# LPD-EPFL/ByzantineMomentum

Measured on AMD Instinct MI355X. Metric: aggregations/sec (Byzantine-robust GAR over n workers x d dims; achieved HBM GB/s per GAR in roofline/per_gar), higher is better.
Workload: dtype f32

## Files before the change

byzantinemomentum_amd/_lib.py:

```python

import ctypes
import pathlib

import torch

import os

_PKG_DIR = pathlib.Path(__file__).resolve().parent
LIB_PATH = pathlib.Path(os.environ["BM_GAR_LIB"]).resolve() if os.environ.get("BM_GAR_LIB") else _PKG_DIR / "libbm_gar.so"

ABI_VERSION = 23
MAX_ROWS = 64
EINVAL = -100000
ENOCOMM, ECOMM = -100001, -100002

OP_MEDIAN, OP_TRMEAN, OP_PHOCAS, OP_MEAMED = 0, 1, 2, 3
WS_PAIRWISE, WS_AKSEL, WS_STATS, WS_DOT, WS_STEP, WS_STUDY = 0, 1, 2, 3, 4, 5
STUDY_SLOTS = 32
STUDY_GRAM, STUDY_EX, STUDY_ATTACK = slice(0, 16), slice(16, 18), slice(18, 20)
STUDY_SUMS = slice(0, 20)
STUDY_MAXES = slice(20, 22)
STUDY_L2 = slice(22, 23)
OUT3_SUMS, OUT3_MAX = slice(0, 2), slice(2, 3)
STEP_S2, STEP_SD, STEP_H2, STEP_HD, STEP_D2, STEP_A2, STEP_AD, STEP_L2 = range(8)
STEP_GRAM, STEP_EX = slice(8, 24), slice(24, 26)
STEP_SMAX, STEP_HMAX, STEP_DMAX, STEP_AMAX = range(26, 30)
STEP_ACCEPT = 30
RANK_KRUM, RANK_BULYAN = 0, 1
ATTACK_EMPIRE, ATTACK_LITTLE, ATTACK_DIRECTION = 0, 1, 16

_c_float_pp = ctypes.POINTER(ctypes.c_void_p)

SIGNATURES = {
  "bm_abi_version": (ctypes.c_int, []),
  "bm_tuning_set": (ctypes.c_int, [ctypes.c_char_p, ctypes.c_int]),
  "bm_error_string": (ctypes.c_char_p, [ctypes.c_int]),
  "bm_colwise": (ctypes.c_int, [ctypes.c_int, _c_float_pp, ctypes.c_int, ctypes.c_int64, ctypes.c_int,
                                ctypes.c_void_p, ctypes.c_void_p]),
  "bm_workspace_bytes": (ctypes.c_int64, [ctypes.c_int, ctypes.c_int, ctypes.c_int64]),
  "bm_pairwise_sqdist": (ctypes.c_int, [_c_float_pp, ctypes.c_int, ctypes.c_int64, ctypes.c_void_p,
                                        ctypes.c_void_p, ctypes.c_void_p]),
  "bm_pairwise_sqdist_shard": (ctypes.c_int, [_c_float_pp, ctypes.c_int, ctypes.c_int64, ctypes.c_int64,
                                              ctypes.c_void_p, ctypes.c_void_p, ctypes.c_void_p]),
  "bm_krum_rank": (ctypes.c_int, [ctypes.c_void_p, ctypes.c_int, ctypes.c_int, ctypes.c_int, ctypes.c_int,
                                  ctypes.c_void_p, ctypes.c_void_p, ctypes.c_void_p]),
  "bm_selected_mean": (ctypes.c_int, [_c_float_pp, ctypes.c_int, ctypes.c_void_p, ctypes.c_int,
                                      ctypes.c_int64, ctypes.c_void_p, ctypes.c_void_p]),
  "bm_bulyan_pass2": (ctypes.c_int, [_c_float_pp, ctypes.c_int, ctypes.c_void_p, ctypes.c_int, ctypes.c_int,
                                     ctypes.c_int64, ctypes.c_void_p, ctypes.c_void_p]),
  "bm_aksel_pass1": (ctypes.c_int, [_c_float_pp, ctypes.c_int, ctypes.c_int64, ctypes.c_void_p,
                                    ctypes.c_void_p, ctypes.c_void_p, ctypes.c_void_p]),
  "bm_stack_stats": (ctypes.c_int, [_c_float_pp, ctypes.c_int, ctypes.c_int64, ctypes.c_void_p, ctypes.c_void_p,
                                    ctypes.c_float, ctypes.c_int, ctypes.c_void_p, ctypes.c_void_p,
                                    ctypes.c_void_p]),
  "bm_multi_dot": (ctypes.c_int, [_c_float_pp, ctypes.c_int, _c_float_pp, ctypes.c_int, ctypes.c_int64,
                                  ctypes.c_void_p, ctypes.c_void_p, ctypes.c_void_p]),
  "bm_momentum_stats_colwise": (ctypes.c_int, [_c_float_pp, ctypes.c_int, _c_float_pp, ctypes.c_int, ctypes.c_int64,
                                               ctypes.c_float, ctypes.c_float, ctypes.c_void_p, ctypes.c_void_p,
                                               ctypes.c_void_p, ctypes.c_void_p, ctypes.c_float, ctypes.c_int,
                                               ctypes.c_int, ctypes.c_int, ctypes.c_int, ctypes.c_void_p,
                                               ctypes.c_void_p, ctypes.c_void_p, ctypes.c_void_p]),
  "bm_momentum_stats_sqdist": (ctypes.c_int, [_c_float_pp, ctypes.c_int, _c_float_pp, ctypes.c_int, ctypes.c_int64,
                                              ctypes.c_int64, ctypes.c_float, ctypes.c_float, ctypes.c_void_p,
                                              ctypes.c_void_p, ctypes.c_void_p, ctypes.c_void_p, ctypes.c_float,
                                              ctypes.c_int, ctypes.c_int, ctypes.c_void_p, ctypes.c_void_p,
                                              ctypes.c_void_p, ctypes.c_void_p, ctypes.c_void_p]),
  "bm_sharded_sq_slot": (ctypes.c_void_p, [ctypes.c_void_p]),
  "bm_sharded_pair_workspace": (ctypes.c_void_p, [ctypes.c_void_p]),
  "bm_sharded_order_slot": (ctypes.c_void_p, [ctypes.c_void_p]),
  "bm_accept_count": (ctypes.c_int, [ctypes.c_void_p, ctypes.c_int, ctypes.c_int, ctypes.c_void_p, ctypes.c_void_p]),
  "bm_sharded_rule_from_sq": (ctypes.c_int, [ctypes.c_void_p, ctypes.c_int, _c_float_pp, ctypes.c_int, ctypes.c_int64,
                                             ctypes.c_int, ctypes.c_int, ctypes.c_void_p, ctypes.c_void_p,
                                             ctypes.c_void_p, ctypes.c_void_p]),
  "bm_stack_stats_colwise": (ctypes.c_int, [_c_float_pp, ctypes.c_int, ctypes.c_int64, ctypes.c_void_p, ctypes.c_void_p,
                                            ctypes.c_float, ctypes.c_int, ctypes.c_int, ctypes.c_int, ctypes.c_int,
                                            ctypes.c_void_p, ctypes.c_void_p, ctypes.c_void_p, ctypes.c_void_p]),
  "bm_stack_stats_sqdist": (ctypes.c_int, [_c_float_pp, ctypes.c_int, ctypes.c_int64, ctypes.c_int64, ctypes.c_void_p,
                                           ctypes.c_void_p, ctypes.c_float, ctypes.c_int, ctypes.c_int, ctypes.c_void_p,
                                           ctypes.c_void_p, ctypes.c_void_p, ctypes.c_void_p, ctypes.c_void_p]),
  "bm_study_stats": (ctypes.c_int, [ctypes.c_void_p, ctypes.c_void_p, ctypes.c_void_p, ctypes.c_void_p, ctypes.c_int,
                                    ctypes.c_void_p, ctypes.c_void_p, ctypes.c_void_p, ctypes.c_void_p, ctypes.c_int,
                                    ctypes.c_float, ctypes.c_float, ctypes.c_void_p, ctypes.c_void_p, ctypes.c_int64,
                                    ctypes.c_void_p, ctypes.c_void_p, ctypes.c_void_p]),
  "bm_study_stats_update": (ctypes.c_int, [ctypes.c_void_p, ctypes.c_void_p, ctypes.c_void_p, ctypes.c_void_p, ctypes.c_int,
                                           ctypes.c_void_p, ctypes.c_void_p, ctypes.c_void_p, ctypes.c_void_p, ctypes.c_int,
                                           ctypes.c_float, ctypes.c_float, ctypes.c_void_p, ctypes.c_void_p,
                                           ctypes.c_void_p, ctypes.c_float, ctypes.c_float, ctypes.c_int64,
                                           ctypes.c_void_p, ctypes.c_void_p, ctypes.c_void_p]),
  "bm_row_sqnorms": (ctypes.c_int, [_c_float_pp, ctypes.c_int, ctypes.c_int64, ctypes.c_void_p, ctypes.c_void_p,
                                    ctypes.c_void_p]),
  "bm_stable_argsort": (ctypes.c_int, [ctypes.c_void_p, ctypes.c_int, ctypes.c_void_p, ctypes.c_void_p]),
  "bm_anticge_workspace_bytes": (ctypes.c_int64, [ctypes.c_int64]),
  "bm_anticge_sum": (ctypes.c_int, [_c_float_pp, ctypes.c_int, ctypes.c_int64, ctypes.c_int, ctypes.c_void_p,
                                    ctypes.c_void_p, ctypes.c_void_p, ctypes.c_void_p, ctypes.c_void_p, ctypes.c_void_p]),
  "bm_anticge_scale": (ctypes.c_int, [ctypes.c_void_p, ctypes.c_int64, ctypes.c_void_p, ctypes.c_void_p]),
  "bm_attack_vector": (ctypes.c_int, [ctypes.c_int, ctypes.c_void_p, ctypes.c_int64, ctypes.c_int64, ctypes.c_float,
                                      ctypes.c_void_p, ctypes.c_void_p, ctypes.c_void_p, ctypes.c_void_p]),
  "bm_multi_axpby": (ctypes.c_int, [_c_float_pp, _c_float_pp, ctypes.c_int, ctypes.c_int64,
                                    ctypes.c_float, ctypes.c_float, ctypes.c_void_p]),
  "bm_brute_select": (ctypes.c_int, [ctypes.c_void_p, ctypes.c_int, ctypes.c_int, ctypes.c_void_p]),
  "bm_momentum_stats": (ctypes.c_int, [_c_float_pp, ctypes.c_int, _c_float_pp, ctypes.c_int, ctypes.c_int64,
                                       ctypes.c_float, ctypes.c_float, ctypes.c_void_p, ctypes.c_void_p,
                                       ctypes.c_void_p, ctypes.c_void_p, ctypes.c_float, ctypes.c_int,
                                       ctypes.c_void_p, ctypes.c_void_p, ctypes.c_void_p]),
  "bm_multi_fma3": (ctypes.c_int, [_c_float_pp, _c_float_pp, _c_float_pp, ctypes.c_int, ctypes.c_int64,
                                   ctypes.c_float, ctypes.c_float, ctypes.c_void_p, ctypes.c_void_p]),
  "bm_multi_fma3_bdev": (ctypes.c_int, [_c_float_pp, _c_float_pp, _c_float_pp, ctypes.c_int, ctypes.c_int64,
                                        ctypes.c_float, ctypes.c_void_p, ctypes.c_void_p, ctypes.c_void_p]),
  "bm_clip_factors": (ctypes.c_int, [ctypes.c_void_p, ctypes.c_int, ctypes.c_float, ctypes.c_void_p,
                                     ctypes.c_void_p]),
  "bm_multi_scale": (ctypes.c_int, [_c_float_pp, ctypes.c_int, ctypes.c_int64, ctypes.c_void_p, ctypes.c_void_p]),
  "bm_comm_available": (ctypes.c_int, []),
  "bm_comm_unique_id": (ctypes.c_int, [ctypes.c_void_p]),
  "bm_comm_init": (ctypes.c_int, [ctypes.POINTER(ctypes.c_void_p), ctypes.c_int, ctypes.c_int, ctypes.c_void_p]),
  "bm_comm_destroy": (ctypes.c_int, [ctypes.c_void_p]),
  "bm_comm_size": (ctypes.c_int, [ctypes.c_void_p]),
  "bm_allreduce_sum_f64": (ctypes.c_int, [ctypes.c_void_p, ctypes.c_void_p, ctypes.c_int64, ctypes.c_void_p]),
  "bm_allgather_f32": (ctypes.c_int, [ctypes.c_void_p, ctypes.c_void_p, ctypes.c_void_p, ctypes.c_int64,
                                      ctypes.c_void_p]),
  "bm_brute_select_device": (ctypes.c_int, [ctypes.c_void_p, ctypes.c_int, ctypes.c_int, ctypes.c_void_p, ctypes.c_void_p,
                                            ctypes.c_void_p]),
  "bm_colwise_eval_supported": (ctypes.c_int, [ctypes.c_int, ctypes.c_int]),
  "bm_colwise_eval_workspace_bytes": (ctypes.c_int64, []),
  "bm_colwise_eval": (ctypes.c_int, [ctypes.c_int, _c_float_pp, ctypes.c_int, ctypes.c_int, ctypes.c_int64, ctypes.c_int,
                                     ctypes.c_void_p, ctypes.c_void_p, ctypes.c_float, ctypes.c_void_p, ctypes.c_void_p,
                                     ctypes.c_void_p]),
  "bm_colwise_eval_tdev": (ctypes.c_int, [ctypes.c_int, _c_float_pp, ctypes.c_int, ctypes.c_int, ctypes.c_int64,
                                          ctypes.c_int, ctypes.c_void_p, ctypes.c_void_p, ctypes.c_void_p, ctypes.c_void_p,
                                          ctypes.c_void_p, ctypes.c_void_p]),
  "bm_sqdist2": (ctypes.c_int, [ctypes.c_void_p, ctypes.c_void_p, ctypes.c_int64, ctypes.c_void_p, ctypes.c_void_p,
                                ctypes.c_void_p]),
  "bm_attack_ranking_device": (ctypes.c_int, [ctypes.c_void_p, ctypes.c_int, ctypes.c_int, ctypes.c_int, ctypes.c_int, ctypes.c_int,
                                              ctypes.c_void_p, ctypes.c_void_p, ctypes.c_void_p]),
  "bm_bulyan_pass2_eval_supported": (ctypes.c_int, [ctypes.c_int, ctypes.c_int, ctypes.c_int]),
  "bm_bulyan_pass2_eval": (ctypes.c_int, [_c_float_pp, ctypes.c_int, ctypes.c_int, ctypes.c_void_p, ctypes.c_int, ctypes.c_int,
                                          ctypes.c_int64, ctypes.c_void_p, ctypes.c_void_p, ctypes.c_float, ctypes.c_void_p,
                                          ctypes.c_void_p, ctypes.c_void_p, ctypes.c_void_p]),
  "bm_order_pair_supported": (ctypes.c_int, [ctypes.c_int]),
  "bm_order_pair": (ctypes.c_int, [_c_float_pp, ctypes.c_int, ctypes.c_int64, ctypes.c_int, ctypes.c_int, ctypes.c_void_p,
                                   ctypes.c_void_p, ctypes.c_void_p]),
  "bm_search_device_next": (ctypes.c_int, [ctypes.c_void_p, ctypes.c_void_p, ctypes.c_int, ctypes.c_int, ctypes.c_double,
                                           ctypes.c_double, ctypes.c_double, ctypes.c_void_p, ctypes.c_void_p,
                                           ctypes.c_void_p]),
  "bm_pairwise_rank": (ctypes.c_int, [_c_float_pp, ctypes.c_int, ctypes.c_int64, ctypes.c_int64, ctypes.c_int, ctypes.c_int,
                                      ctypes.c_int, ctypes.c_void_p, ctypes.c_void_p, ctypes.c_void_p, ctypes.c_void_p,
                                      ctypes.c_void_p]),
  "bm_sharded_workspace_bytes": (ctypes.c_int64, [ctypes.c_int, ctypes.c_int64]),
  "bm_sharded_krum": (ctypes.c_int, [ctypes.c_void_p, _c_float_pp, ctypes.c_int, ctypes.c_int64, ctypes.c_int64,
                                     ctypes.c_int, ctypes.c_int, ctypes.c_void_p, ctypes.c_void_p, ctypes.c_void_p, ctypes.c_void_p]),
  "bm_sharded_bulyan": (ctypes.c_int, [ctypes.c_void_p, _c_float_pp, ctypes.c_int, ctypes.c_int64, ctypes.c_int64,
                                       ctypes.c_int, ctypes.c_int, ctypes.c_void_p, ctypes.c_void_p, ctypes.c_void_p,
                                       ctypes.c_void_p]),
  "bm_step_stats_count": (ctypes.c_int, []),
  "bm_step_workspace_bytes": (ctypes.c_int64, [ctypes.c_int, ctypes.c_int64]),
  "bm_step_worker": (ctypes.c_int, [ctypes.c_void_p, ctypes.c_void_p, _c_float_pp, _c_float_pp, ctypes.c_int64,
                                    ctypes.c_int64] + [ctypes.c_void_p] * 13),
  "bm_search_begin": (ctypes.c_int, [ctypes.c_void_p, ctypes.c_double, ctypes.c_double, ctypes.c_double]),
  "bm_search_propose": (ctypes.c_int, [ctypes.c_void_p, ctypes.c_void_p]),
  "bm_search_report": (ctypes.c_int, [ctypes.c_void_p, ctypes.c_double]),
  "bm_attack_objective": (ctypes.c_int, [ctypes.c_void_p, ctypes.c_int, ctypes.c_int, ctypes.c_int, ctypes.c_int,
                                         ctypes.c_int, ctypes.c_double, ctypes.c_void_p, ctypes.c_void_p,
                                         ctypes.c_void_p]),
  "bm_attack_line_search": (ctypes.c_int, [ctypes.c_void_p, ctypes.c_int, ctypes.c_int, ctypes.c_int, ctypes.c_int,
                                           ctypes.c_int, ctypes.c_int, ctypes.c_int, ctypes.c_void_p, ctypes.c_void_p]),
  "bm_attack_line_search_device": (ctypes.c_int, [ctypes.c_void_p, ctypes.c_int, ctypes.c_int, ctypes.c_int,
                                                  ctypes.c_int, ctypes.c_int, ctypes.c_int, ctypes.c_int,
                                                  ctypes.c_void_p, ctypes.c_void_p]),
  "bm_attack_ranking": (ctypes.c_int, [ctypes.c_void_p, ctypes.c_int, ctypes.c_int, ctypes.c_int, ctypes.c_int,
                                       ctypes.c_int, ctypes.c_double, ctypes.c_void_p]),
}

class Search(ctypes.Structure):
  _fields_ = [("best_x", ctypes.c_double), ("best_y", ctypes.c_double), ("probe", ctypes.c_double),
              ("step", ctypes.c_double), ("ratio", ctypes.c_double), ("phase", ctypes.c_int32),
              ("evaluations", ctypes.c_int32), ("awaiting", ctypes.c_int32), ("reserved", ctypes.c_int32)]


ATTACK_VECTOR_KINDS = {"nan": 0, "shift_one": 1, "shift_all": 2, "scale": 3}
RULE_IDS = {"krum": 0, "bulyan": 1, "median": 2, "trmean": 3, "phocas": 4, "meamed": 5, "brute": 6, "average": 7}


class StepParams(ctypes.Structure):
  _fields_ = [("n", ctypes.c_int32), ("f_decl", ctypes.c_int32), ("f_real", ctypes.c_int32), ("ks", ctypes.c_int32),
              ("rule", ctypes.c_int32), ("m", ctypes.c_int32), ("attack_kind", ctypes.c_int32),
              ("nb_past", ctypes.c_int32), ("past_count", ctypes.c_int32), ("attack_scale", ctypes.c_float),
              ("mu", ctypes.c_float), ("one_minus_damp", ctypes.c_float), ("clip", ctypes.c_float),
              ("oldest_weight", ctypes.c_float)]


class NativeLibraryError(RuntimeError):
  """libbm_gar.so is missing, stale or failed to load: the HIP path cannot run."""


_lib = None


def load():
  global _lib
  if _lib is not None:
    return _lib
  if not LIB_PATH.exists():
    raise NativeLibraryError(
      f"{LIB_PATH} not found: build it with `python -m byzantinemomentum_amd.build` "
      "(hipcc --offload-arch=gfx950). There is no CPU fallback.")
  try:
    lib = ctypes.CDLL(str(LIB_PATH))
  except OSError as err:
    raise NativeLibraryError(f"cannot load {LIB_PATH}: {err}") from err
  for name, (restype, argtypes) in SIGNATURES.items():
    try:
      fn = getattr(lib, name)
    except AttributeError as err:
      raise NativeLibraryError(f"{LIB_PATH} does not export {name!r} (stale build?)") from err
    fn.restype = restype
    fn.argtypes = argtypes
  if lib.bm_abi_version() != ABI_VERSION:
    raise NativeLibraryError(
      f"{LIB_PATH} has ABI {lib.bm_abi_version()}, host code expects {ABI_VERSION}: rebuild")
  _lib = lib
  return lib


def check(code, what):
  if code != 0:
    msg = load().bm_error_string(code).decode("utf-8", "replace")
    raise RuntimeError(f"libbm_gar {what} failed: {msg} (code {code})")


def pointer_table(tensors):
  arr = (ctypes.c_void_p * len(tensors))()
  for i, t in enumerate(tensors):
    arr[i] = t.data_ptr()
  return arr
```

byzantinemomentum_amd/csrc/api.cpp:

```cpp
#include <stdlib.h>
#include <string.h>
#include <math.h>
#include <algorithm>
#include <vector>
#include "bm_common.h"

namespace bm {
static int env_int(const char* name, int dflt) {
  const char* v = getenv(name);
  if (v == nullptr || *v == '\0') return dflt;
  return atoi(v);
}
static double env_double(const char* name, double dflt) {
  const char* v = getenv(name);
  if (v == nullptr || *v == '\0') return dflt;
  return atof(v);
}
Tuning& tuning_mutable() {
  static Tuning t = {env_int("BM_COL_BURST", 8),  env_int("BM_MEAN_BURST", 8),
                           env_int("BM_STEP_BURST", 8), env_int("BM_STEP_STREAM", 0), env_int("BM_PAIR_MODE", 0),
                           env_int("BM_PAIR_PLANES", 0), env_int("BM_PAIR_DITHER", 0), env_double("BM_PAIR_TAU", 2e-3),
                           env_int("BM_STUDY_BURST", 8), env_int("BM_STEP_STAGGER_US", 0),
                           env_int("BM_GRAM_STEADY", 1), env_int("BM_BULYAN_SHORT", 1),
                           env_int("BM_PAIR_LOAD_NT", 1), env_int("BM_RANK_ALGO", 0), env_int("BM_COL_WIDE", 1), env_int("BM_BRUTE_BUDGET", 0)};
  return t;
}
const Tuning& tuning() { return tuning_mutable(); }
}

extern "C" int bm_abi_version(void) { return 23; }

extern "C" int bm_tuning_set(const char* name, int value) {
  using namespace bm;
  if (name == nullptr) return BM_EINVAL;
  Tuning& t = tuning_mutable();
  const struct { const char* key; int* slot; } knobs[] = {
      {"BM_COL_BURST", &t.col_burst}, {"BM_MEAN_BURST", &t.mean_burst}, {"BM_STEP_BURST", &t.step_burst},
      {"BM_STEP_STREAM", &t.step_stream}, {"BM_PAIR_MODE", &t.pair_mode}, {"BM_PAIR_PLANES", &t.pair_planes},
      {"BM_PAIR_DITHER", &t.pair_dither}, {"BM_STUDY_BURST", &t.study_burst},
      {"BM_STEP_STAGGER_US", &t.step_stagger_us}, {"BM_GRAM_STEADY", &t.gram_steady},
      {"BM_BULYAN_SHORT", &t.bulyan_short}, {"BM_PAIR_LOAD_NT", &t.pair_load_nt},
      {"BM_RANK_ALGO", &t.rank_algo}, {"BM_COL_WIDE", &t.col_wide}, {"BM_BRUTE_BUDGET", &t.brute_budget}};
  for (const auto& k : knobs)
    if (strcmp(name, k.key) == 0) {
      *k.slot = value;
      return 0;
    }
  return BM_EINVAL;
}

extern "C" const char* bm_error_string(int code) {
  if (code == 0) return "success";
  if (code == BM_EINVAL) return "invalid argument for libbm_gar";
  if (code == BM_ENOCOMM) return "RCCL is not available in this process (librccl.so.1 could not be bound)";
  if (code == BM_ECOMM) return "an RCCL call failed";
  if (code < 0) return hipGetErrorString(static_cast<hipError_t>(-code));
  return "unknown libbm_gar status";
}

namespace {
struct BruteGraph {
  int n;
  uint64_t adj[BM_MAX_ROWS];

  void build(const double* dist, double t) {
    for (int i = 0; i < n; ++i) adj[i] = 0;
    for (int i = 0; i < n; ++i)
      for (int j = i + 1; j < n; ++j) {
        const double v = dist[i * n + j];
        if (isfinite(v) && v <= t) {
          adj[i] |= (uint64_t)1 << j;
          adj[j] |= (uint64_t)1 << i;
        }
      }
  }

  bool has_clique(uint64_t cand, int need) const {
    const int count = __builtin_popcountll(cand);
    if (count < need) return false;
    if (need <= 1) return true;
    int worst = -1, worst_missing = 0;
    for (uint64_t rest = cand; rest != 0; rest &= rest - 1) {
      const int u = __builtin_ctzll(rest);
      const int missing = __builtin_popcountll(cand & ~adj[u] & ~((uint64_t)1 << u));
      if (missing > worst_missing) {
        worst = u;
        worst_missing = missing;
      }
    }
    if (worst < 0) return true;
    const int budget = count - need;
    if (budget == 0) return false;
    const uint64_t bit = (uint64_t)1 << worst;
    if (worst_missing <= budget && has_clique(cand & (adj[worst] | bit), need)) return true;
    return has_clique(cand & ~bit, need);
  }
};
}

extern "C" int bm_brute_select(const double* dist_nxn, int n, int f, int32_t* sel_out) {
  if (dist_nxn == nullptr || sel_out == nullptr || n < 1 || n > BM_MAX_ROWS || f < 0 || n - f < 1)
    return BM_EINVAL;
  const int k = n - f;
  const uint64_t everyone = n == 64 ? ~(uint64_t)0 : (((uint64_t)1 << n) - 1);
  std::vector<double> values;
  values.reserve((size_t)n * (n - 1) / 2 + 1);
  values.push_back(0.0);
  for (int i = 0; i < n; ++i)
    for (int j = i + 1; j < n; ++j) {
      const double v = dist_nxn[i * n + j];
      if (isfinite(v) && v > 0.0) values.push_back(v);
    }
  std::sort(values.begin(), values.end());
  values.erase(std::unique(values.begin(), values.end()), values.end());
  BruteGraph g;
  g.n = n;
  g.build(dist_nxn, values.back());
  if (!g.has_clique(everyone, k)) return BM_EINVAL;
  size_t lo = 0, hi = values.size() - 1;
  while (lo < hi) {
    const size_t mid = (lo + hi) / 2;
    g.build(dist_nxn, values[mid]);
    if (g.has_clique(everyone, k))
      hi = mid;
    else
      lo = mid + 1;
  }
  g.build(dist_nxn, values[lo]);
  uint64_t cand = everyone;
  int chosen = 0;
  for (int c = 0; c < n && chosen < k; ++c) {
    const uint64_t bit = (uint64_t)1 << c;
    if ((cand & bit) == 0) continue;
    const uint64_t above = c == 63 ? 0 : ~(((uint64_t)1 << (c + 1)) - 1);
    const uint64_t next = cand & g.adj[c] & above;
    if (g.has_clique(next, k - chosen - 1)) {
      sel_out[chosen++] = c;
      cand = next;
    }
  }
  return chosen == k ? 0 : BM_EINVAL;
}
```

byzantinemomentum_amd/csrc/bm_common.h:

```cpp
#pragma once
#include <hip/hip_runtime.h>
#include <stdint.h>
#include <utility>
#include "../../include/bm_gar.h"
#include "launch_plan.h"

namespace bm {

struct RowTable {
  const float* p[BM_MAX_ROWS];
  RowTable advanced(int64_t by) const {
    RowTable t = *this;
    advance(t.p, by);
    return t;
  }
};

static inline int hip_code(hipError_t e) { return e == hipSuccess ? 0 : -(int)e; }

#define BM_LAUNCH_CHECK()                      \
  do {                                         \
    hipError_t e__ = hipGetLastError();        \
    if (e__ != hipSuccess) return hip_code(e__); \
  } while (0)

template <int N>
struct MergeExchange {
  static constexpr int kMax = (N < 2) ? 1 : (N * 10);
  struct Table {
    short a[kMax];
    short b[kMax];
    int count;
  };
  static constexpr Table make() {
    Table t{};
    t.count = 0;
    if (N < 2) return t;
    int tt = 0;
    while ((1 << tt) < N) ++tt;
    for (int p = 1 << (tt - 1); p > 0; p /= 2) {
      int q = 1 << (tt - 1), r = 0, d = p;
      while (true) {
        for (int i = 0; i < N - d; ++i)
          if ((i & p) == r) {
            t.a[t.count] = (short)i;
            t.b[t.count] = (short)(i + d);
            ++t.count;
          }
        if (q == p) break;
        d = q - p;
        q /= 2;
        r = p;
      }
    }
    return t;
  }
  static constexpr Table table = make();
};

__device__ __forceinline__ void cmp_exchange(float& a, float& b) {
  float lo, hi;
  asm("v_min_f32 %0, %1, %2" : "=v"(lo) : "v"(a), "v"(b));
  asm("v_max_f32 %0, %1, %2" : "=v"(hi) : "v"(a), "v"(b));
  a = lo;
  b = hi;
}

template <int N, size_t... I>
__device__ __forceinline__ void sort_network_impl(float (&x)[N], std::index_sequence<I...>) {
  (cmp_exchange(x[MergeExchange<N>::table.a[I]], x[MergeExchange<N>::table.b[I]]), ...);
}

template <int N>
__device__ __forceinline__ void sort_network(float (&x)[N]) {
  if constexpr (N >= 2)
    sort_network_impl<N>(x, std::make_index_sequence<MergeExchange<N>::table.count>{});
}

__device__ __forceinline__ float div_small_int(float x, float m, float rm) {
  const float q = x * rm;
  const float r = __builtin_fmaf(-q, m, x);
  const float q1 = __builtin_fmaf(r, rm, q);
  return (q1 == q1) ? q1 : q;
}

template <int VEC>
struct VecLoad;
template <>
struct VecLoad<4> {
  using T = float __attribute__((ext_vector_type(4)));
};
template <>
struct VecLoad<2> {
  using T = float __attribute__((ext_vector_type(2)));
};
template <>
struct VecLoad<1> {
  using T = float;
};

template <int VEC>
__device__ __forceinline__ void load_stream(const float* p, float (&dst)[VEC]) {
  using T = typename VecLoad<VEC>::T;
  const T v = __builtin_nontemporal_load(reinterpret_cast<const T*>(p));
  if constexpr (VEC == 1) {
    dst[0] = v;
  } else {
#pragma unroll
    for (int c = 0; c < VEC; ++c) dst[c] = v[c];
  }
}

template <int VEC>
__device__ __forceinline__ void load_stream_off(const float* base, uint32_t byte_off, float (&dst)[VEC]) {
  load_stream<VEC>(reinterpret_cast<const float*>(reinterpret_cast<const char*>(base) + byte_off), dst);
}

template <int VEC>
__device__ __forceinline__ void store_stream_off(float* base, uint32_t byte_off, const float (&src)[VEC]);

template <int VEC>
__device__ __forceinline__ void store_stream(float* p, const float (&src)[VEC]) {
  using T = typename VecLoad<VEC>::T;
  T v;
  if constexpr (VEC == 1) {
    v = src[0];
  } else {
#pragma unroll
    for (int c = 0; c < VEC; ++c) v[c] = src[c];
  }
  __builtin_nontemporal_store(v, reinterpret_cast<T*>(p));
}

template <int VEC>
__device__ __forceinline__ void store_stream_off(float* base, uint32_t byte_off, const float (&src)[VEC]) {
  store_stream<VEC>(reinterpret_cast<float*>(reinterpret_cast<char*>(base) + byte_off), src);
}

template <int VEC>
__device__ __forceinline__ void store_result(float* p, const float (&src)[VEC]) {
  using T = typename VecLoad<VEC>::T;
  T v;
  if constexpr (VEC == 1) {
    v = src[0];
  } else {
#pragma unroll
    for (int c = 0; c < VEC; ++c) v[c] = src[c];
  }
  *reinterpret_cast<T*>(p) = v;
}
template <int VEC>
__device__ __forceinline__ void store_result_off(float* base, uint32_t byte_off, const float (&src)[VEC]) {
  store_result<VEC>(reinterpret_cast<float*>(reinterpret_cast<char*>(base) + byte_off), src);
}
template <int VEC>
__device__ __forceinline__ void store_result_policy(float* p, const float (&src)[VEC], int nt) {
  if (nt)
    store_stream<VEC>(p, src);
  else
    store_result<VEC>(p, src);
}

constexpr int kColMaxBlocks = 256 * 64;

static inline int lds_opt_in(const void* kernel, size_t dynamic_bytes, size_t static_bytes) {
  if (dynamic_bytes + static_bytes <= 48u * 1024u) return 0;
  return hip_code(hipFuncSetAttribute(kernel, hipFuncAttributeMaxDynamicSharedMemorySize, (int)dynamic_bytes));
}

static inline int compute_units() {
  static int cached[16] = {0};
  int dev = 0;
  if (hipGetDevice(&dev) != hipSuccess || dev < 0 || dev >= 16) dev = 0;
  if (cached[dev] == 0) {
    int cus = 0;
    if (hipDeviceGetAttribute(&cus, hipDeviceAttributeMultiprocessorCount, dev) != hipSuccess || cus <= 0) cus = 256;
    cached[dev] = cus;
  }
  return cached[dev];
}

__device__ __forceinline__ bool arrive_last(int* counter, int total, int* lds_flag) {
  asm volatile("s_waitcnt vmcnt(0)" ::: "memory");
  __syncthreads();
  if (threadIdx.x == 0) {
    __builtin_amdgcn_fence(__ATOMIC_RELEASE, "agent");
    asm volatile("s_waitcnt vmcnt(0)" ::: "memory");
    const int ticket = atomicAdd(counter, 1);
    const int last = (ticket == total - 1) ? 1 : 0;
    if (last) __builtin_amdgcn_fence(__ATOMIC_ACQUIRE, "agent");
    *lds_flag = last;
  }
  __syncthreads();
  return *lds_flag != 0;
}

__device__ __forceinline__ int32_t load_index_coherent(const int32_t* p) {
  return __hip_atomic_load(p, __ATOMIC_RELAXED, __HIP_MEMORY_SCOPE_AGENT);
}

template <int BLOCK>
__device__ __forceinline__ double block_reduce_sum(double v, double* lds ) {
#pragma unroll
  for (int off = 32; off > 0; off >>= 1) v += __shfl_down(v, off, 64);
  const int wave = threadIdx.x >> 6, lane = threadIdx.x & 63;
  if (lane == 0) lds[wave] = v;
  __syncthreads();
  double r = 0.0;
  if (threadIdx.x == 0) {
#pragma unroll
    for (int w = 0; w < BLOCK / 64; ++w) r += lds[w];
  }
  __syncthreads();
  return r;
}

__device__ __forceinline__ float byzantine_coordinate(float avg, float q, float fk, float scale, int attack_kind) {
  const float dir = ((attack_kind & 15) == BM_ATTACK_LITTLE) ? __builtin_sqrtf(q / (fk - 1.0f)) : -avg;
  const float att = dir * scale;
  return (attack_kind & BM_ATTACK_DIRECTION) ? att : avg + att;
}

}

namespace bm {
struct Tuning {
  int col_burst;
  int mean_burst;
  int step_burst;
  int step_stream;
  int pair_mode;
  int pair_planes;
  int pair_dither;
  double pair_tau;
  int study_burst;
  int step_stagger_us;
  int gram_steady;
  int bulyan_short;
  int pair_load_nt;
  int rank_algo;
  int col_wide;
  int brute_budget;
};
const Tuning& tuning();
Tuning& tuning_mutable();
}
```

byzantinemomentum_amd/csrc/linesearch.cpp:

```cpp
#include <algorithm>
#include <cmath>
#include <cstdint>
#include <vector>

#include "bm_common.h"
#include "search_core.h"

extern "C" int bm_brute_select(const double* dist_nxn, int n, int f, int32_t* sel_out);

namespace {

using namespace bm;

struct AttackGeometry {
  int h, k, n;
  std::vector<double> a;
  std::vector<double> w;
  std::vector<double> uu;
  std::vector<double> hh;
  double c;

  AttackGeometry(const double* ext, int h_, int k_) : h(h_), k(k_), n(h_ + k_), a(h_), w(h_), uu((size_t)h_ * h_), hh((size_t)h_ * h_) {
    const int e = h + 2;
    c = ext[h * e + h + 1];
    for (int i = 0; i < h; ++i) {
      a[i] = ext[i * e + h];
      w[i] = attack_w(a[i], c, ext[i * e + h + 1]);
    }
    for (int i = 0; i < h; ++i)
      for (int j = 0; j < h; ++j) {
        hh[(size_t)i * h + j] = ext[i * e + j];
        uu[(size_t)i * h + j] = attack_uu(a[i], a[j], ext[i * e + j], i == j);
      }
  }

  void sqdist(double t, std::vector<double>& sq) const {
    sq.assign((size_t)n * n, 0.0);
    for (int i = 0; i < h; ++i) {
      for (int j = 0; j < h; ++j) sq[(size_t)i * n + j] = hh[(size_t)i * h + j];
      const double q = attack_candidate_sq(a[i], w[i], c, t);
      for (int j = h; j < n; ++j) {
        sq[(size_t)i * n + j] = q;
        sq[(size_t)j * n + i] = q;
      }
    }
  }

  double objective(const std::vector<int>& sel_sorted, double t) const {
    int kb = 0;
    bool on[BM_MAX_ROWS] = {false};
    for (int i : sel_sorted) {
      if (i >= h) ++kb;
      else on[i] = true;
    }
    double rows[BM_MAX_ROWS] = {0.0}, ws[BM_MAX_ROWS] = {0.0};
    const int span = attack_row_span(h);
    for (int i = 0; i < h; ++i) {
      if (!on[i]) continue;
      ws[i] = w[i];
      double lo = 0.0, hi = 0.0;
      for (int j = 0; j < span / 2; ++j) lo += (j < h && on[j]) ? uu[(size_t)i * h + j] : 0.0;
      for (int j = span / 2; j < span; ++j) hi += (j < h && on[j]) ? uu[(size_t)i * h + j] : 0.0;
      rows[i] = lo + hi;
    }
    return attack_objective_value(butterfly_order_sum(rows), butterfly_order_sum(ws), kb, t, c, (int)sel_sorted.size());
  }
};

void rank_order(const std::vector<double>& sq, int n, int take, std::vector<int>& order) {
  std::vector<double> score(n), row;
  take = std::max(0, std::min(take, n - 1));
  for (int i = 0; i < n; ++i) {
    row.clear();
    for (int j = 0; j < n; ++j) {
      if (j == i) continue;
      double v = std::sqrt(sq[(size_t)i * n + j]);
      if (!std::isfinite(v)) v = INFINITY;
      row.push_back(v);
    }
    std::sort(row.begin(), row.end());
    double s = 0.0;
    for (int t = 0; t < take; ++t) s += row[t];
    score[i] = s;
  }
  order.resize(n);
  for (int i = 0; i < n; ++i) order[i] = i;
  std::stable_sort(order.begin(), order.end(), [&](int x, int y) { return score[x] < score[y]; });
}

int select(const AttackGeometry& g, int f, int rule, int m, double t, std::vector<int>& sel) {
  const int n = g.n;
  std::vector<double> sq;
  if (rule == BM_RULE_AVERAGE) {
    sel.resize(n);
    for (int i = 0; i < n; ++i) sel[i] = i;
    return 0;
  }
  g.sqdist(t, sq);
  if (rule == BM_RULE_KRUM) {
    std::vector<int> order;
    rank_order(sq, n, n - f - 1, order);
    sel.assign(order.begin(), order.begin() + m);
    return 0;
  }
  for (double& v : sq) v = std::sqrt(v);
  std::vector<int32_t> out(n - f);
  const int rc = bm_brute_select(sq.data(), n, f, out.data());
  if (rc != 0) return rc;
  sel.assign(out.begin(), out.end());
  return 0;
}

bool valid(const double* ext, int h, int k, int f, int rule, int& m) {
  const int n = h + k;
  if (ext == nullptr || h < 1 || k < 0 || n > BM_MAX_ROWS || f < 0) return false;
  if (rule == BM_RULE_KRUM) {
    if (m <= 0) m = n - f - 2;
    return m >= 1 && m <= n;
  }
  if (rule == BM_RULE_BRUTE) return n - f >= 1;
  return rule == BM_RULE_AVERAGE;
}

}

extern "C" int bm_search_begin(bm_search* c, double start, double delta, double ratio) {
  if (c == nullptr || !(start >= 0.0) || !(delta > 0.0) || !(ratio > 0.5 && ratio < 1.0)) return BM_EINVAL;
  cursor_begin(c, start, delta, ratio);
  return 0;
}

extern "C" int bm_search_propose(bm_search* c, double* x_out) {
  if (c == nullptr || x_out == nullptr || c->awaiting) return BM_EINVAL;
  cursor_propose(c);
  c->awaiting = 1;
  *x_out = c->probe;
  return 0;
}

extern "C" int bm_search_report(bm_search* c, double y) {
  if (c == nullptr || !c->awaiting) return BM_EINVAL;
  cursor_report(c, y);
  c->awaiting = 0;
  return 0;
}

extern "C" int bm_attack_objective(const double* ext, int h, int k, int f, int rule, int m, double t,
                                   double* y_out, int32_t* sel_out, int32_t* count_out) {
  if (!valid(ext, h, k, f, rule, m) || y_out == nullptr) return BM_EINVAL;
  const AttackGeometry g(ext, h, k);
  std::vector<int> sel;
  const int rc = select(g, f, rule, m, t, sel);
  if (rc != 0) return rc;
  if (sel_out != nullptr)
    for (size_t i = 0; i < sel.size(); ++i) sel_out[i] = sel[i];
  if (count_out != nullptr) *count_out = (int32_t)sel.size();
  std::sort(sel.begin(), sel.end());
  *y_out = g.objective(sel, t);
  return 0;
}

extern "C" int bm_attack_ranking(const double* ext, int h, int k, int f, int mode, int m, double t,
                                 int32_t* order_out) {
  const int n = h + k;
  if (ext == nullptr || order_out == nullptr || h < 1 || k < 0 || n > BM_MAX_ROWS || f < 0 ||
      (mode != BM_RANK_KRUM && mode != BM_RANK_BULYAN))
    return BM_EINVAL;
  if (m <= 0) m = n - f - 2;
  if (m < 1 || m > n) return BM_EINVAL;
  const AttackGeometry g(ext, h, k);
  std::vector<double> sq;
  g.sqdist(t, sq);
  std::vector<int> order;
  rank_order(sq, n, mode == BM_RANK_KRUM ? n - f - 1 : m, order);
  for (int i = 0; i < n; ++i) order_out[i] = order[i];
  return 0;
}

extern "C" int bm_attack_line_search(const double* ext, int h, int k, int f, int rule, int m, int evals,
                                     int negative, double* factor_out, double* trace_out) {
  if (!valid(ext, h, k, f, rule, m) || factor_out == nullptr || evals < 1) return BM_EINVAL;
  const AttackGeometry g(ext, h, k);
  std::vector<int> sel;
  bm_search cur;
  int rc = bm_search_begin(&cur, 0.0, 1.0, 0.8);
  for (int e = 0; e < evals && rc == 0; ++e) {
    double x = 0.0;
    rc = bm_search_propose(&cur, &x);
    if (rc != 0) break;
    const double t = negative ? -x : x;
    rc = select(g, f, rule, m, t, sel);
    if (rc != 0) break;
    std::sort(sel.begin(), sel.end());
    const double y = g.objective(sel, t);
    if (trace_out != nullptr) {
      trace_out[2 * e] = x;
      trace_out[2 * e + 1] = y;
    }
    rc = bm_search_report(&cur, y);
  }
  *factor_out = cur.best_x;
  return rc;
}
```

byzantinemomentum_amd/csrc/search_core.h:

```cpp
#pragma once
#include "bm_common.h"

namespace bm {

enum { kSearchFirst = 0, kSearchGrow = 1, kSearchShrink = 2 };

__host__ __device__ inline void cursor_begin(bm_search* c, double start, double delta, double ratio) {
  c->best_x = start;
  c->best_y = 0.0;
  c->probe = start;
  c->step = delta;
  c->ratio = ratio;
  c->phase = kSearchFirst;
  c->evaluations = 0;
  c->awaiting = 0;
  c->reserved = 0;
}

__host__ __device__ inline void cursor_propose(bm_search* c) {
  switch (c->phase) {
    case kSearchFirst:
      break;
    case kSearchGrow:
      c->probe = c->best_x + c->step;
      break;
    default:
      if (c->probe < c->best_x) {
        c->probe += c->step;
      } else {
        double x = c->probe - c->step;
        while (x < 0.0) x = 0.5 * (x + c->probe);
        c->probe = x;
      }
  }
}

__host__ __device__ inline void cursor_report(bm_search* c, double y) {
  const bool better = (c->phase == kSearchFirst) || (y > c->best_y);
  if (better) {
    c->best_x = c->probe;
    c->best_y = y;
  }
  switch (c->phase) {
    case kSearchFirst:
      c->phase = kSearchGrow;
      break;
    case kSearchGrow:
      if (better) {
        c->step *= 2.0;
      } else {
        c->step *= c->ratio;
        c->phase = kSearchShrink;
      }
      break;
    default:
      c->step *= c->ratio;
  }
  ++c->evaluations;
}

__host__ __device__ inline double attack_w(double a_i, double c, double ext_i_att) { return 0.5 * (a_i + c - ext_i_att); }
__host__ __device__ inline double attack_uu(double a_i, double a_j, double ext_ij, bool same) {
  return same ? a_i : 0.5 * (a_i + a_j - ext_ij);
}
__host__ __device__ inline double attack_candidate_sq(double a_i, double w_i, double c, double t) {
  const double q = a_i - 2.0 * t * w_i + t * t * c;
  return (q < 0.0) ? 0.0 : q;
}
__host__ __device__ inline int attack_row_span(int h) { return (h + 7) & ~7; }
inline double butterfly_order_sum(const double (&slots)[BM_MAX_ROWS]) {
  double cur[BM_MAX_ROWS], nxt[BM_MAX_ROWS];
  for (int i = 0; i < BM_MAX_ROWS; ++i) cur[i] = slots[i];
  for (int s = 1; s < BM_MAX_ROWS; s <<= 1) {
    for (int i = 0; i < BM_MAX_ROWS; ++i) nxt[i] = cur[i] + cur[i ^ s];
    for (int i = 0; i < BM_MAX_ROWS; ++i) cur[i] = nxt[i];
  }
  return cur[0];
}

__host__ __device__ inline double attack_objective_value(double quad, double lin, int kb, double t, double c, int count) {
  const double cnt = (double)count;
  return (quad + 2.0 * kb * t * lin + (double)kb * kb * t * t * c) / (cnt * cnt);
}

}
```

byzantinemomentum_amd/csrc/search_device.hip:

```cpp
#include <cstdlib>

#include "bm_common.h"
#include "rank_body.h"
#include "search_core.h"

namespace bm {

constexpr int kSearchBlock = 1024;
constexpr int kSearchWaves = kSearchBlock / 64;
constexpr int kSortRowsPerWave = BM_MAX_ROWS / kSearchWaves;
constexpr int kRankChunk = BM_MAX_ROWS / kSearchWaves;
constexpr int kByzWave = 1;

__host__ __device__ inline int search_ld(int h) { return attack_row_span(h) + 1; }
__host__ __device__ inline size_t search_lds_bytes(int h) {
  return (size_t)(2 * h * search_ld(h) + 2 * BM_MAX_ROWS + 2) * sizeof(double) +
         (size_t)2 * kSearchWaves * BM_MAX_ROWS * sizeof(int);
}

__device__ __forceinline__ double lane_value(double v, int src) {
  const long long bits = __double_as_longlong(v);
  const unsigned lo = (unsigned)__builtin_amdgcn_readlane((int)(unsigned)bits, src);
  const unsigned hi = (unsigned)__builtin_amdgcn_readlane((int)(unsigned)((unsigned long long)bits >> 32), src);
  return __longlong_as_double((long long)(((unsigned long long)hi << 32) | lo));
}

__device__ __forceinline__ int rank_share(double v, int lane, int first, int count) {
  int before = 0;
#pragma unroll
  for (int q = 0; q < kRankChunk; ++q) {
    const int j = first + q;
    const double o = lane_value(v, j < count ? j : 0);
    before += (j < count && (o < v || (o == v && j < lane))) ? 1 : 0;
  }
  return before;
}

__device__ __forceinline__ int longest(int v, int limit) {
  if (__builtin_amdgcn_ballot_w64(v >= limit) != 0ull) return limit;
  unsigned long long among = ~0ull;
  int most = 0;
#pragma unroll
  for (int bit = 5; bit >= 0; --bit) {
    const unsigned long long with = __builtin_amdgcn_ballot_w64(((v >> bit) & 1) != 0) & among;
    if (with != 0ull) {
      among = with;
      most |= 1 << bit;
    }
  }
  return most;
}

__device__ __forceinline__ double butterfly_sum(double v) {
#pragma unroll
  for (int s = 1; s < 64; s <<= 1) v = v + __shfl_xor(v, s, 64);
  return v;
}

constexpr int kTraceSlots = 12;
template <bool TRACE, bool RANKING = false>
__global__ __launch_bounds__(kSearchBlock) void attack_search_kernel(const double* __restrict__ ext, int h, int k, int f,
                                                                     int rule, int m, int evals, int negative,
                                                                     double* __restrict__ out, const double* __restrict__ t_dev,
                                                                     int32_t* __restrict__ order_out, int take_arg) {
  constexpr bool ranking = RANKING;
  const unsigned long long clock0 = TRACE ? __builtin_amdgcn_s_memtime() : 0ull;
  extern __shared__ double search_smem[];
  const int n = h + k, e = h + 2, tid = threadIdx.x, ld = search_ld(h);
  const int wave = __builtin_amdgcn_readfirstlane(tid >> 6), lane = tid & 63;
  auto stamp = [&](int ev, int slot) {
    if (TRACE && lane == 0 && wave <= kByzWave)
      out[1 + 2 * evals + (2 * ev + wave) * kTraceSlots + slot] = (double)(__builtin_amdgcn_s_memtime() - clock0);
  };
  double* const UU = search_smem;
  double* const HS = UU + h * ld;
  double* const SC = HS + h * ld;
  double* const Q = SC + BM_MAX_ROWS;
  double* const Y = Q + BM_MAX_ROWS;
  int* const PART = reinterpret_cast<int*>(Y + 2);
  int* const PARTQ = PART + kSearchWaves * BM_MAX_ROWS;
  const double c = ext[h * e + h + 1];
  const double kInf = __builtin_inf();
  const bool krum = rule == BM_RULE_KRUM;

  for (int p = tid; p < h * h; p += kSearchBlock) {
    const int i = p / h, j = p - i * h;
    UU[i * ld + j] = attack_uu(ext[i * e + h], ext[j * e + h], ext[i * e + j], i == j);
  }
  if (krum) {
    double sorted[kSortRowsPerWave];
#pragma unroll
    for (int r = 0; r < kSortRowsPerWave; ++r) {
      const int i = wave + r * kSearchWaves;
      sorted[r] = (i < h && lane < h && lane != i) ? rank_distance(ext[i * e + lane]) : kInf;
    }
#pragma unroll
    for (int kk = 2; kk <= 64; kk <<= 1) {
#pragma unroll
      for (int j = kk >> 1; j > 0; j >>= 1) {
        const bool keep_min = ((lane & kk) == 0) == ((lane & j) == 0);
#pragma unroll
        for (int r = 0; r < kSortRowsPerWave; ++r) {
          const double o = __shfl_xor(sorted[r], j, 64);
          sorted[r] = keep_min ? __builtin_fmin(sorted[r], o) : __builtin_fmax(sorted[r], o);
        }
      }
    }
#pragma unroll
    for (int r = 0; r < kSortRowsPerWave; ++r) {
      const int i = wave + r * kSearchWaves;
      if (i < h && lane < h - 1) HS[i * ld + lane] = sorted[r];
    }
  }
  const bool honest = lane < h;
  const double a = honest ? ext[lane * e + h] : 0.0;
  const double w = honest ? attack_w(a, c, ext[lane * e + h + 1]) : 0.0;
  const double* const uu = UU + (honest ? lane : 0) * ld;
  const double* const hs = HS + (honest ? lane : 0) * ld;
  int take = take_arg >= 0 ? take_arg : n - f - 1;
  take = take > n - 1 ? n - 1 : take;
  take = take < 0 ? 0 : take;
  const int count = krum ? m : n;
  const int hm1 = h - 1, last = hm1 > 0 ? hm1 - 1 : 0, span = attack_row_span(h);
  const unsigned long long honest_rows = (h >= 64) ? ~0ull : ((1ull << h) - 1ull);
  unsigned long long selected = (n >= 64) ? ~0ull : ((1ull << n) - 1ull);
  double row = 0.0;
  __syncthreads();
  stamp(0, 11);

  bm_search cur;
  cursor_begin(&cur, 0.0, 1.0, 0.8);
  for (int ev = 0; ev < evals; ++ev) {
    cursor_propose(&cur);
    const double x = cur.probe;
    const double t = ranking ? t_dev[0] : (negative ? -x : x);
    stamp(ev, 0);
    if (krum) {
      const double dq = honest ? rank_distance(attack_candidate_sq(a, w, c, t)) : kInf;
      if (k > 0) {
        PARTQ[wave * BM_MAX_ROWS + lane] = rank_share(dq, lane, wave * kRankChunk, h);
        __syncthreads();
      }
      stamp(ev, 1);
      if (wave == 0) {
        int below = 0, len = hm1;
#pragma unroll
        for (int it = 0; it < 6; ++it) {
          const int half = len >> 1, mid = below + half;
          const double v = hs[mid < hm1 ? mid : last];
          const bool right = len > 0 && v < dq;
          below = right ? mid + 1 : below;
          len = right ? len - half - 1 : half;
        }
        stamp(ev, 2);
        const int b1 = below < take ? below : take;
        const int c2 = (take - b1 < k) ? take - b1 : k;
        const int c3 = take - b1 - c2;
        const int most1 = longest(b1, take), most3 = longest(c3, take);
        double score = 0.0;
        for (int u0 = 0; u0 < most1; u0 += 8) {
          double g[8];
#pragma unroll
          for (int q = 0; q < 8; ++q) g[q] = hs[u0 + q];
#pragma unroll
          for (int q = 0; q < 8; ++q) score += (u0 + q < b1) ? g[q] : 0.0;
        }
        if (__builtin_amdgcn_ballot_w64(c2 > 0) != 0ull) {
          for (int u = 0; u < k; ++u) score += (u < c2) ? dq : 0.0;
        }
        const double* const hs3 = hs + b1;
        for (int u0 = 0; u0 < most3; u0 += 8) {
          double g[8];
#pragma unroll
          for (int q = 0; q < 8; ++q) g[q] = hs3[u0 + q];
#pragma unroll
          for (int q = 0; q < 8; ++q) score += (u0 + q < c3) ? g[q] : 0.0;
        }
        if (honest) SC[lane] = score;
      } else if (wave == kByzWave && k > 0) {
        int place = 0;
#pragma unroll
        for (int q = 0; q < kSearchWaves; ++q) place += PARTQ[q * BM_MAX_ROWS + lane];
        if (honest) Q[place] = dq;
        __builtin_amdgcn_fence(__ATOMIC_RELEASE, "wavefront");
        __builtin_amdgcn_wave_barrier();
        __builtin_amdgcn_fence(__ATOMIC_ACQUIRE, "wavefront");
        stamp(ev, 2);
        const int zeros = (k - 1 < take) ? k - 1 : take;
        const int rest = take - zeros;
        double sb = 0.0;
#pragma unroll 8
        for (int u = 0; u < rest; ++u) sb += Q[u];
        if (lane < k) SC[h + lane] = sb;
      }
      stamp(ev, 3);
      __syncthreads();
      stamp(ev, 4);
      if (lane < n) {
        const double si = SC[lane];
        int before = 0;
#pragma unroll
        for (int q = 0; q < kRankChunk; ++q) {
          const int j = wave * kRankChunk + q;
          const double sj = SC[j < n ? j : 0];
          before += (j < n && (sj < si || (sj == si && j < lane))) ? 1 : 0;
        }
        PART[wave * BM_MAX_ROWS + lane] = before;
      }
      __syncthreads();
      stamp(ev, 5);
    }
    if (wave == 0) {
      if (krum) {
        int rank = 0;
#pragma unroll
        for (int q = 0; q < kSearchWaves; ++q) rank += PART[q * BM_MAX_ROWS + (lane < n ? lane : 0)];
        selected = __builtin_amdgcn_ballot_w64(lane < n && rank < m);
        if (ranking) {
          int* const inv = reinterpret_cast<int*>(SC);
          inv[lane] = 0;
          __builtin_amdgcn_fence(__ATOMIC_RELEASE, "wavefront");
          __builtin_amdgcn_wave_barrier();
          __builtin_amdgcn_fence(__ATOMIC_ACQUIRE, "wavefront");
          if (lane < n && rank < BM_MAX_ROWS) inv[rank] = lane;
          __builtin_amdgcn_fence(__ATOMIC_RELEASE, "wavefront");
          __builtin_amdgcn_wave_barrier();
          __builtin_amdgcn_fence(__ATOMIC_ACQUIRE, "wavefront");
          order_out[lane] = lane < n ? inv[lane] : 0;
        }
      }
      stamp(ev, 6);
      if (!ranking && (krum || ev == 0)) {
        const unsigned long long on = selected & honest_rows;
        const int half = span >> 1;
        double lo = 0.0, hi = 0.0;
        for (int j0 = 0; j0 < half; j0 += 4) {
          double g[4], gh[4];
#pragma unroll
          for (int q = 0; q < 4; ++q) {
            g[q] = uu[j0 + q];
            gh[q] = uu[half + j0 + q];
          }
#pragma unroll
          for (int q = 0; q < 4; ++q) {
            lo += ((on >> (j0 + q)) & 1ull) ? g[q] : 0.0;
            hi += ((on >> (half + j0 + q)) & 1ull) ? gh[q] : 0.0;
          }
        }
        row = lo + hi;
      }
      stamp(ev, 7);
      const bool mine = honest && ((selected >> lane) & 1ull);
      const double quad = butterfly_sum(mine ? row : 0.0), lin = butterfly_sum(mine ? w : 0.0);
      stamp(ev, 8);
      const int kb = __builtin_popcountll(h >= 64 ? 0ull : (selected >> h));
      const double y = attack_objective_value(quad, lin, kb, t, c, count);
      if (lane == 0 && !ranking) {
        out[1 + 2 * ev] = x;
        out[2 + 2 * ev] = y;
        Y[0] = y;
      }
      stamp(ev, 9);
    }
    __syncthreads();
    if (!ranking) cursor_report(&cur, Y[0]);
    stamp(ev, 10);
  }
  if (tid == 0 && !ranking) out[0] = cur.best_x;
}

__global__ void search_cursor_kernel(bm_search* __restrict__ state, const double* __restrict__ y, int negative, int last,
                                     double start, double delta, double ratio, double* __restrict__ t_out,
                                     double* __restrict__ out) {
  bm_search cur;
  if (y == nullptr) {
    cursor_begin(&cur, start, delta, ratio);
  } else {
    cur = *state;
    out[2 + 2 * cur.evaluations] = y[0];
    cursor_report(&cur, y[0]);
  }
  if (last) {
    out[0] = cur.best_x;
  } else {
    cursor_propose(&cur);
    out[1 + 2 * cur.evaluations] = cur.probe;
    t_out[0] = negative ? -cur.probe : cur.probe;
  }
  *state = cur;
}

}

extern "C" int bm_search_device_next(void* state, const double* y, int negative, int last, double start, double delta,
                                     double ratio, double* t_out, double* out, void* stream) {
  using namespace bm;
  if (state == nullptr || out == nullptr || (!last && t_out == nullptr) || (last && y == nullptr)) return BM_EINVAL;
  if (y == nullptr && (!(start >= 0.0) || !(delta > 0.0) || !(ratio > 0.5 && ratio < 1.0))) return BM_EINVAL;
  hipLaunchKernelGGL(search_cursor_kernel, dim3(1), dim3(1), 0, static_cast<hipStream_t>(stream),
                     static_cast<bm_search*>(state), y, negative ? 1 : 0, last ? 1 : 0, start, delta, ratio, t_out, out);
  BM_LAUNCH_CHECK();
  return 0;
}

extern "C" int bm_attack_line_search_device(const double* ext, int h, int k, int f, int rule, int m, int evals,
                                            int negative, double* out, void* stream) {
  using namespace bm;
  const int n = h + k;
  if (ext == nullptr || out == nullptr || h < 1 || k < 0 || n > BM_MAX_ROWS || f < 0 || evals < 1) return BM_EINVAL;
  if (rule == BM_RULE_KRUM) {
    if (m <= 0) m = n - f - 2;
    if (m < 1 || m > n) return BM_EINVAL;
  } else if (rule != BM_RULE_AVERAGE) {
    return BM_EINVAL;
  }
  const size_t lds = search_lds_bytes(h);
  const char* trace_env = getenv("BM_SEARCH_TRACE");
  const bool trace = trace_env != nullptr && trace_env[0] == '1';
  auto kernel = trace ? attack_search_kernel<true> : attack_search_kernel<false>;
  const int rc = lds_opt_in(reinterpret_cast<const void*>(kernel), lds, 0);
  if (rc != 0) return rc;
  hipLaunchKernelGGL(kernel, dim3(1), dim3(kSearchBlock), lds, static_cast<hipStream_t>(stream), ext, h, k, f, rule, m, evals,
                     negative ? 1 : 0, out, static_cast<const double*>(nullptr), static_cast<int32_t*>(nullptr), -1);
  BM_LAUNCH_CHECK();
  return 0;
}

extern "C" int bm_attack_ranking_device(const double* ext, int h, int k, int f, int mode, int m, const double* t_dev,
                                        int32_t* order_out, void* stream) {
  using namespace bm;
  const int n = h + k;
  if (ext == nullptr || order_out == nullptr || t_dev == nullptr || h < 1 || k < 1 || n > BM_MAX_ROWS || f < 0 ||
      (mode != BM_RANK_KRUM && mode != BM_RANK_BULYAN))
    return BM_EINVAL;
  if (m <= 0) m = n - f - 2;
  if (m < 1 || m > n) return BM_EINVAL;
  const int take = mode == BM_RANK_KRUM ? n - f - 1 : m;
  const size_t lds = search_lds_bytes(h);
  auto kernel = attack_search_kernel<false, true>;
  const int rc = lds_opt_in(reinterpret_cast<const void*>(kernel), lds, 0);
  if (rc != 0) return rc;
  hipLaunchKernelGGL(kernel, dim3(1), dim3(kSearchBlock), lds, static_cast<hipStream_t>(stream), ext, h, k, f, (int)BM_RULE_KRUM,
                     m, 1, 0, static_cast<double*>(nullptr), t_dev, order_out, take);
  BM_LAUNCH_CHECK();
  return 0;
}
```

byzantinemomentum_amd/linesearch.py:

```python

import ctypes

import torch

from . import _lib

ANALYTIC_RULES = ("krum", "brute", "average")


def line_maximize(scape, evals=16, start=0., delta=1., ratio=0.8):
  lib = _lib.load()
  if not isinstance(evals, int) or evals < 1:
    _lib.check(_lib.EINVAL, "line_maximize (evals must be a positive integer)")
  cursor = _lib.Search()
  _lib.check(lib.bm_search_begin(ctypes.byref(cursor), start, delta, ratio), "bm_search_begin")
  x = ctypes.c_double()
  trace = []
  for _ in range(evals):
    _lib.check(lib.bm_search_propose(ctypes.byref(cursor), ctypes.byref(x)), "bm_search_propose")
    y = float(scape(x.value))
    trace.append((x.value, y))
    _lib.check(lib.bm_search_report(ctypes.byref(cursor), y), "bm_search_report")
  return cursor.best_x, trace


def _ext_pointer(ext, h):
  if not (isinstance(ext, torch.Tensor) and ext.dtype == torch.float64 and ext.device.type == "cpu"
          and ext.is_contiguous() and tuple(ext.shape) == (h + 2, h + 2)):
    raise ValueError(f"ext must be a contiguous float64 CPU tensor of shape ({h + 2}, {h + 2})")
  return ctypes.c_void_p(ext.data_ptr())


def attack_objective(ext, h, k, f, rule, t, m=None):
  lib = _lib.load()
  y = ctypes.c_double()
  sel = (ctypes.c_int32 * _lib.MAX_ROWS)()
  count = ctypes.c_int32()
  _lib.check(lib.bm_attack_objective(_ext_pointer(ext, h), h, k, f, _lib.RULE_IDS[rule], m or 0, float(t),
                                     ctypes.cast(ctypes.pointer(y), ctypes.c_void_p),
                                     ctypes.cast(sel, ctypes.c_void_p),
                                     ctypes.cast(ctypes.pointer(count), ctypes.c_void_p)), "bm_attack_objective")
  return y.value, list(sel[:count.value])


def attack_ranking(ext, h, k, f, mode, t, m=None):
  lib = _lib.load()
  order = (ctypes.c_int32 * _lib.MAX_ROWS)()
  mode_id = {"krum": _lib.RANK_KRUM, "bulyan": _lib.RANK_BULYAN}[mode]
  _lib.check(lib.bm_attack_ranking(_ext_pointer(ext, h), h, k, f, mode_id, m or 0, float(t),
                                   ctypes.cast(order, ctypes.c_void_p)), "bm_attack_ranking")
  return list(order[:h + k])


def attack_line_search(ext, h, k, f, rule, evals=16, negative=False, m=None):
  if rule not in ANALYTIC_RULES:
    raise ValueError(f"no scalar form of the search for rule {rule!r}")
  lib = _lib.load()
  factor = ctypes.c_double()
  trace = (ctypes.c_double * (2 * evals))()
  _lib.check(lib.bm_attack_line_search(_ext_pointer(ext, h), h, k, f, _lib.RULE_IDS[rule], m or 0, evals,
                                       1 if negative else 0, ctypes.cast(ctypes.pointer(factor), ctypes.c_void_p),
                                       ctypes.cast(trace, ctypes.c_void_p)), "bm_attack_line_search")
  return factor.value, [(trace[2 * i], trace[2 * i + 1]) for i in range(evals)]
```

byzantinemomentum_amd/sharded.py:

```python

import ctypes
import math
import warnings

import torch
import torch.distributed as dist

from . import _lib

__all__ = ["shard_bounds", "owned_workers", "Shards", "ShardedAggregator", "HipBackend", "NativeComm"]


class Shards(list):

  def __init__(self, rows=(), d_total=None):
    super().__init__(rows)
    self.d_total = None if d_total is None else int(d_total)


def shard_bounds(d, world_size, rank, align=64):
  per = -(-d // world_size)
  per = -(-per // align) * align
  lo = min(rank * per, d)
  hi = min(lo + per, d)
  return lo, hi


def owned_workers(n, world_size, rank):
  return list(range(rank, n, world_size))


class NativeComm:

  def __init__(self, group=None, vote=None):
    lib = _lib.load()
    if not lib.bm_comm_available():
      raise RuntimeError("RCCL could not be bound by libbm_gar.so")
    world, rank = dist.get_world_size(group), dist.get_rank(group)
    ident, failure = [None], None
    if rank == 0:
      try:
        buf = ctypes.create_string_buffer(128)
        _lib.check(lib.bm_comm_unique_id(buf), "bm_comm_unique_id")
        ident[0] = buf.raw
      except Exception as err:
        failure = err
    if vote is not None:
      if not vote(failure is None):
        raise RuntimeError(f"bm_comm_unique_id failed on rank 0: {failure}" if failure is not None else
                           "bm_comm_unique_id failed on rank 0")
    elif failure is not None:
      raise failure
    dist.broadcast_object_list(ident, src=dist.get_global_rank(group, 0) if group is not None else 0, group=group)
    handle = ctypes.c_void_p()
    _lib.check(lib.bm_comm_init(ctypes.byref(handle), world, rank, ctypes.c_char_p(ident[0])), "bm_comm_init")
    self.handle = handle
    self.world_size = world

  def close(self):
    if self.handle is not None and self.handle.value:
      _lib.load().bm_comm_destroy(self.handle)
      self.handle = None

  def __del__(self):
    try:
      self.close()
    except Exception:
      pass


class HipBackend:

  capabilities = frozenset((
    "step_worker", "momentum_stats_colwise", "momentum_stats_sqdist", "stack_stats_colwise", "stack_stats_sqdist",
    "device_search", "attack_ranking_device", "bulyan_pass2_eval", "order_pair", "colwise_eval", "sqdist2", "anticge",
    "accept_count", "attack_vector"))

  def __init__(self):
    from . import gars, stats
    self.gars = gars
    self.stats = stats


  def pairwise_sqdist(self, gradients, d_total=None):
    return self.gars.pairwise_sqdist(gradients, d_total)

  def rank(self, sq, n, f, m, mode):
    order, _ = self.gars.rank_from_sqdist(sq, n, f, m, mode)
    return order

  def selected_mean(self, gradients, order, m):
    return self.gars.selected_mean(gradients, order, m)

  def bulyan_pass2(self, gradients, order, f, m):
    return self.gars.bulyan_pass2(gradients, order, f, m)

  def colwise(self, rule, gradients, f):
    return getattr(self.gars, rule)(gradients, f=f) if rule != "median" else self.gars.median(gradients)

  def aksel_sqdist(self, gradients):
    return self.gars.aksel_sqdist(gradients)[:len(gradients)]

  def argsort(self, keys, n):
    return self.gars.stable_argsort(keys, n)

  def brute_select(self, dist_host, n, f):
    return self.gars.brute_select_host(dist_host, n, f)

  def brute_select_device(self, sq, n, f):
    return self.gars.brute_select_device(sq, n, f)

  def sharded_rule(self, name, comm, gradients, f, m, d_total=None, with_order=False):
    gars = self.gars
    n, d, device = gars._validate(gradients)
    lib = _lib.load()
    out = torch.empty(d, dtype=torch.float32, device=device)
    nbytes = lib.bm_sharded_workspace_bytes(n, d)
    ws = gars._Scratch.get(device, "ws_sharded", nbytes=int(nbytes))
    fn = lib.bm_sharded_krum if name == "krum" else lib.bm_sharded_bulyan
    with torch.cuda.device(device):
      _lib.check(fn(comm.handle if comm is not None else None, _lib.pointer_table(gradients), n, d,
                    int(d_total) if d_total is not None else d, f, m, gars._ptr(out), None, gars._ptr(ws), gars._stream(device)), "bm_sharded_" + name)
    if with_order:
      at = lib.bm_sharded_order_slot(gars._ptr(ws)) - ws.data_ptr()
      return out, ws[at:at + 4 * _lib.MAX_ROWS].view(torch.int32)
    return out

  def index_tensor(self, indices, like):
    return torch.tensor(indices, dtype=torch.int32, device=like.device)

  def sum_over_ranks(self, agg, value):
    t = torch.tensor([float(value)], dtype=torch.float64, device=torch.device("cuda", torch.cuda.current_device()))
    return int(agg.all_reduce_sum(t).item())


  def stack_stats(self, samples, scale=None, attack="empire", want_avg=True, direction=False):
    return self.stats.stack_stats_async(samples, scale=scale, attack=attack, want_avg=want_avg, direction=direction)

  def momentum_stats(self, sampled, buffers, mu, omd, factors, scale, attack, direction=False):
    return self.stats.momentum_stats(sampled, buffers, mu, omd, factors, scale, attack, direction)

  def momentum_stats_colwise(self, *args, **kwargs):
    return self.stats.momentum_stats_colwise(*args, **kwargs)

  def stack_stats_colwise(self, *args, **kwargs):
    return self.stats.stack_stats_colwise(*args, **kwargs)

  def stack_stats_sqdist(self, *args, **kwargs):
    return self.stats.stack_stats_sqdist(*args, **kwargs)

  def momentum_stats_sqdist(self, *args, **kwargs):
    return self.stats.momentum_stats_sqdist(*args, **kwargs)

  def multi_fma3(self, outs, ps, qs, a, b, p_scale=None):
    return self.stats.multi_fma3(outs, ps, qs, a, b, p_scale)

  @property
  def device_search_rules(self):
    return self.stats.DEVICE_SEARCH_RULES

  def attack_search_device(self, *args, **kwargs):
    return self.stats.attack_search_device(*args, **kwargs)

  def device_search(self, device, evals, negative=False):
    return self.stats.DeviceSearch(device, evals, negative)

  def multi_scale(self, ys, factors):
    return self.stats.multi_scale(ys, factors)

  def row_sqnorms(self, gradients):
    return self.stats.row_sqnorms(gradients).contiguous()

  def clip_factors_from_sq(self, sq, k, clip):
    return self.stats.clip_factors_from_sq(sq, k, clip)

  def study_stats(self, *args, **kwargs):
    return self.stats.study_stats(*args, **kwargs)

  def accept_count(self, order, count, h):
    return self.stats.accept_count(order, count, h)

  def anticge(self, honests, f_decl, reduce):
    byz, _, scal = self.stats.anticge_sum(honests, f_decl, reduce(self.row_sqnorms(honests)))
    reduce(scal[:1])
    return self.stats.anticge_scale(byz, scal)

  def attack_vector(self, kind, h_avg, factor=None, target=None, want_direction=False):
    return self.stats.attack_vector(kind, h_avg, factor, target, want_direction)

  def colwise_eval_supported(self, rule, n):
    return self.stats.colwise_eval_supported(rule, n)

  def colwise_eval(self, *args, **kwargs):
    return self.stats.colwise_eval(*args, **kwargs)

  def sqdist2(self, a, b):
    return self.stats.sqdist2(a, b)

  def attack_ranking_device(self, *args, **kwargs):
    return self.stats.attack_ranking_device(*args, **kwargs)

  def bulyan_pass2_eval_supported(self, n, f, m, d=0):
    return self.stats.bulyan_pass2_eval_supported(n, f, m, d)

  def bulyan_pass2_eval(self, *args, **kwargs):
    return self.stats.bulyan_pass2_eval(*args, **kwargs)

  def order_pair_supported(self, h):
    return self.stats.order_pair_supported(h)

  def order_pair(self, rows, il, ih):
    return self.stats.order_pair(rows, il, ih)

  def study_dots(self, core, extra):
    return self.stats.study_dots(core, extra)

  def step_worker(self, comm, *args, **kwargs):
    return self.stats.step_worker(comm, *args, **kwargs)


def _anticge_sum_torch(backend, local, f_decl, sq):
  h = len(local)
  maxpos = h - f_decl
  keys = torch.where(torch.isfinite(sq[:h]), sq[:h], torch.full_like(sq[:h], math.inf))
  order = backend.argsort(keys, h)
  ranked = order[:h].tolist()
  attack = local[ranked[0]].clone()
  for i in ranked[:maxpos]:
    attack.add_(local[i])
  return attack, order, torch.stack([attack.double().pow(2).sum(), keys[ranked[maxpos]]])


def _anticge_scale_torch(vec, scal):
  attnorm, byznorm = scal.sqrt().float().tolist()
  if attnorm > 0:
    vec.mul_(-math.nextafter(byznorm, 0) / attnorm)
  return vec


def _attack_vector_torch(kind, avg, factor, target, want_direction):
  if kind == "nan":
    return torch.full_like(avg, math.nan)
  if isinstance(factor, torch.Tensor):
    factor = factor.reshape(-1)[0].to(avg.device, torch.float32)
  else:
    factor = torch.tensor(float(factor), dtype=torch.float32, device=avg.device)
  if kind == "scale":
    return avg * factor
  direction = torch.ones_like(avg) if kind == "shift_all" else torch.zeros_like(avg)
  if kind == "shift_one" and target is not None and target >= 0:
    direction[target] = 1
  out = avg + factor * direction
  return (out, direction) if want_direction else out


class ShardedAggregator:

  def __init__(self, backend=None, group=None, force_collectives=False, native_comm="auto", local_only=False):
    self.backend = backend if backend is not None else HipBackend()
    self.group = group
    initialised = dist.is_available() and dist.is_initialized() and not local_only
    self.world_size = dist.get_world_size(group) if initialised else 1
    self.rank = dist.get_rank(group) if initialised else 0
    self.collective = self.world_size > 1 or (force_collectives and initialised)
    self.native = None
    self.single_call = isinstance(self.backend, HipBackend) and native_comm is not False
    if self.single_call and self.collective:
      self.native, failure = self._create_native(group)
      if self.native is None:
        if native_comm is True:
          raise RuntimeError(f"libbm_gar RCCL communicator unavailable on at least one rank ({failure})")
        warnings.warn(f"libbm_gar RCCL communicator unavailable ({failure}); using torch.distributed collectives")
        self.single_call = False
    self.brute_status = None
    self.last_selection = None
    self._total = None

  def shard_rows(self, rows, d=None):
    d = int(rows[0].shape[0]) if d is None else int(d)
    lo, hi = shard_bounds(d, self.world_size, self.rank)
    return Shards([r[lo:hi] for r in rows], d_total=d)

  def _total_of(self, local, d_total=None):
    if d_total is None:
      d_total = getattr(local, "d_total", None)
    return self.total_length(local[0].numel(), d_total)

  def total_length(self, d_local, d_total=None):
    if d_total is not None:
      return int(d_total)
    if not self.collective:
      return int(d_local)
    if self._total is None:
      self._total = (int(self.backend.sum_over_ranks(self, int(d_local))), int(d_local))
    elif self._total[1] != int(d_local):
      raise ValueError(f"this ShardedAggregator determined the total length {self._total[0]} from shards of "
                       f"{self._total[1]} coordinates and is now given a shard of {d_local}: pass d_total=, or call "
                       f"reset_total_length() on every rank")
    return self._total[0]

  def reset_total_length(self):
    self._total = None

  def _create_native(self, group):
    lib = _lib.load()

    def everyone(ok):
      flag = torch.tensor([1.0 if ok else 0.0], dtype=torch.float32,
                          device=torch.device("cuda", torch.cuda.current_device()))
      dist.all_reduce(flag, op=dist.ReduceOp.MIN, group=group)
      return flag.item() >= 1.0

    if not everyone(bool(lib.bm_comm_available())):
      return None, "RCCL could not be bound by libbm_gar.so"
    comm, failure = None, None
    try:
      comm = NativeComm(group, vote=everyone)
    except Exception as err:
      failure = err
    if not everyone(comm is not None):
      if comm is not None:
        comm.close()
      return None, failure if failure is not None else "bm_comm_init failed on another rank"
    return comm, None


  def _all_reduce(self, tensor, op=None):
    if self.collective:
      dist.all_reduce(tensor, op=(op or dist.ReduceOp.SUM), group=self.group)
    return tensor

  def _all_gather_into(self, everyone, mine):
    dist.all_gather_into_tensor(everyone, mine, group=self.group)

  def _all_to_all(self, recv, send):
    dist.all_to_all_single(recv, send, group=self.group)

  def all_reduce_sum(self, tensor):
    return self._all_reduce(tensor)

  def exchange(self, sums, maxes):
    if not self.collective:
      return sums, maxes
    ns = sums.shape[0]
    mine = torch.cat([sums, maxes]).contiguous()
    everyone = torch.empty(self.world_size * mine.shape[0], dtype=mine.dtype, device=mine.device)
    self._all_gather_into(everyone, mine)
    everyone = everyone.view(self.world_size, -1)
    total = everyone[0, :ns].clone()
    for r in range(1, self.world_size):
      total += everyone[r, :ns]
    return total, everyone[:, ns:].max(dim=0).values

  def all_gather_output(self, local_out, d):
    if not self.collective:
      return local_out
    lo0, hi0 = shard_bounds(d, self.world_size, 0)
    per = hi0 - lo0
    padded = torch.zeros(per, dtype=local_out.dtype, device=local_out.device)
    padded[:local_out.shape[0]] = local_out
    full = torch.empty(per * self.world_size, dtype=local_out.dtype, device=local_out.device)
    self._all_gather_into(full, padded)
    return full[:d]

  def to_dim_sharded(self, my_gradients, n, d, dtype=torch.float32, device=None):
    world, rank = self.world_size, self.rank
    mine = owned_workers(n, world, rank)
    if len(my_gradients) != len(mine):
      raise ValueError(f"rank {rank} must pass the gradients of workers {mine}")
    if not self.collective:
      return Shards(my_gradients, d_total=d)
    per = -(-(-(-d // world)) // 64) * 64
    n_max = -(-n // world)
    if my_gradients:
      dtype, device = my_gradients[0].dtype, my_gradients[0].device
    elif device is None:
      device = torch.device("cuda", torch.cuda.current_device()) if torch.cuda.is_available() else torch.device("cpu")
    send = torch.zeros((world, n_max, per), dtype=dtype, device=device)
    for j, g in enumerate(my_gradients):
      full = g.shape[0] // per
      send[:full, j, :] = g[:full * per].view(full, per)
      if full < world and g.shape[0] > full * per:
        send[full, j, :g.shape[0] - full * per] = g[full * per:]
    recv = torch.empty_like(send)
    self._all_to_all(recv.view(-1), send.view(-1))
    lo, hi = shard_bounds(d, world, rank)
    return Shards([recv[i % world, i // world, :hi - lo] for i in range(n)], d_total=d)


  def median(self, local):
    return self.backend.colwise("median", local, 0)

  def trmean(self, local, f):
    return self.backend.colwise("trmean", local, f)

  def phocas(self, local, f):
    return self.backend.colwise("phocas", local, f)

  def meamed(self, local, f):
    return self.backend.colwise("meamed", local, f)

  def global_sqdist(self, local, d_total=None):
    sq = self.backend.pairwise_sqdist(local, d_total=self._total_of(local, d_total))
    self._all_reduce(sq)
    return sq

  def krum(self, local, f, m=None, d_total=None):
    n = len(local)
    if m is None:
      m = n - f - 2
    if self.single_call:
      out, order = self.backend.sharded_rule("krum", self.native, local, f, m, self._total_of(local, d_total),
                                             with_order=True)
      self.last_selection = (order, m)
      return out
    order = self.backend.rank(self.global_sqdist(local, d_total), n, f, m, _lib.RANK_KRUM)
    self.last_selection = (order, m)
    return self.backend.selected_mean(local, order, m)

  def bulyan(self, local, f, m=None, d_total=None):
    n = len(local)
    if m is None:
      m = n - f - 2
    if self.single_call:
      return self.backend.sharded_rule("bulyan", self.native, local, f, m, self._total_of(local, d_total))
    order = self.backend.rank(self.global_sqdist(local, d_total), n, f, m, _lib.RANK_BULYAN)
    return self.backend.bulyan_pass2(local, order, f, m)

  def rule_from_sq(self, name, local, local_sq, f, m=None):
    n = len(local)
    if m is None:
      m = n - f - 2
    sq = self._all_reduce(local_sq)
    order = self.backend.rank(sq, n, f, m, _lib.RANK_KRUM if name == "krum" else _lib.RANK_BULYAN)
    if name == "krum":
      self.last_selection = (order, m)
      return self.backend.selected_mean(local, order, m)
    return self.backend.bulyan_pass2(local, order, f, m)

  def aksel(self, local, f, mode="mid"):
    n = len(local)
    count = (n + 1) // 2 if mode == "mid" else n - f
    sq = self.backend.aksel_sqdist(local)
    self._all_reduce(sq)
    order = self.backend.argsort(sq, n)
    self.last_selection = (order, count)
    return self.backend.selected_mean(local, order, count)

  def brute(self, local, f, d_total=None, check=False):
    n = len(local)
    sq = self.global_sqdist(local, d_total)
    if hasattr(self.backend, "brute_select_device"):
      sel, self.brute_status = self.backend.brute_select_device(sq, n, f)
      if check and not (sq.is_cuda and torch.cuda.is_current_stream_capturing()):
        code = int(self.brute_status.item())
        if code == -2:
          host = self.backend.brute_select(sq.sqrt().cpu().contiguous(), n, f)
          sel = self.backend.index_tensor(host, local[0])
          self.brute_status = None
        elif code != 0:
          from . import gars
          raise RuntimeError(gars.BRUTE_NO_SUBSET)
      self.last_selection = (sel, n - f)
      return self.backend.selected_mean(local, sel, n - f)
    self.brute_status = None
    sel = self.backend.index_tensor(self.backend.brute_select(sq.sqrt().cpu().contiguous(), n, f), local[0])
    self.last_selection = (sel, n - f)
    return self.backend.selected_mean(local, sel, n - f)

  def check_brute(self):
    status = getattr(self, "brute_status", None)
    if status is not None:
      from . import gars
      gars.brute_check(status)

  def average(self, local):
    n = len(local)
    return self.backend.selected_mean(local, self.backend.index_tensor(list(range(n)), local[0]), n)

  def cge(self, local, f):
    n = len(local)
    sq = self.backend.row_sqnorms(local)
    self._all_reduce(sq)
    order = self.backend.argsort(sq, n)
    self.last_selection = (order, n - f)
    return self.backend.selected_mean(local, order, n - f)

  def anticge(self, local_honests, f_decl, f_real):
    local = list(local_honests)
    h = len(local)
    if f_real <= 0:
      return []
    if f_real > f_decl:
      return [torch.full_like(local[0], math.nan)] * f_real
    if not 1 <= f_decl <= h:
      raise ValueError(f"anticge needs 1 <= f_decl <= {h} honest gradients, got f_decl = {f_decl}")
    if "anticge" in getattr(self.backend, "capabilities", ()):
      return [self.backend.anticge(local, f_decl, self._all_reduce)] * f_real
    byz, _, scal = _anticge_sum_torch(self.backend, local, f_decl, self._all_reduce(self.backend.row_sqnorms(local)))
    self._all_reduce(scal[:1])
    return [_anticge_scale_torch(byz, scal)] * f_real

  def attack_vector(self, kind, local_avg, factor=None, target_idx=None, d_total=None, want_direction=False):
    if kind not in _lib.ATTACK_VECTOR_KINDS:
      raise ValueError(f"unknown attack vector kind {kind!r} (one of {sorted(_lib.ATTACK_VECTOR_KINDS)})")
    if want_direction and kind not in ("shift_one", "shift_all"):
      raise ValueError(f"kind {kind!r} has no direction vector")
    target = None
    if kind == "shift_one":
      if not isinstance(target_idx, int) or isinstance(target_idx, bool):
        raise ValueError(f"kind 'shift_one' needs an integer target_idx, got {target_idx!r}")
      total = self.total_length(local_avg.numel(), d_total)
      if not -total <= target_idx < total:
        raise IndexError(f"index {target_idx} is out of bounds for dimension 0 with size {total}")
      lo, hi = shard_bounds(total, self.world_size, self.rank)
      where = target_idx % total
      target = where - lo if lo <= where < hi else -1
    if "attack_vector" in getattr(self.backend, "capabilities", ()):
      return self.backend.attack_vector(kind, local_avg, factor, target, want_direction)
    return _attack_vector_torch(kind, local_avg, factor, target, want_direction)

  def compute_avg_dev_max(self, local_samples):
    k = len(local_samples)
    if k == 0:
      return None, math.nan, math.nan, math.nan
    avg, out3 = self.backend.stack_stats(local_samples)
    sums, mx = self.exchange(out3[:2], out3[2:])
    norm2, dev2 = sums.tolist()
    amax = mx.item()
    dev = math.sqrt(dev2 / (k - 1)) if k >= 2 else math.nan
    return avg, math.sqrt(norm2), dev, amax
```

byzantinemomentum_amd/stats.py:

```python

import ctypes
import os
import math

import torch

from . import _lib
from . import gars

__all__ = ["compute_avg_dev_max", "stack_stats_async", "study_dots", "study_stats", "multi_axpby", "row_sqnorms", "momentum_stats", "momentum_stats_colwise", "momentum_stats_sqdist", "stack_stats_colwise", "stack_stats_sqdist",
           "multi_fma3", "clip_factors", "clip_factors_from_sq", "multi_scale", "clip_gradients", "l2_distance",
           "step_worker", "anticge_sum", "anticge_scale", "anticge_attack", "accept_count",
           "attack_vector", "nan_attack", "bulyan_attack", "empire_strict_attack"]

_ptr = gars._ptr


def _opt(t):
  return _ptr(t) if t is not None else None


def _require_scalar_on(t, device, message):
  if not (isinstance(t, torch.Tensor) and t.is_cuda and t.device == device and t.dtype == torch.float64
          and t.numel() >= 1 and t.is_contiguous()):
    raise gars.GarInputError(message)


def _require_ext(ext, h):
  if not (isinstance(ext, torch.Tensor) and ext.is_cuda and ext.dtype == torch.float64 and ext.is_contiguous()
          and tuple(ext.shape) == (h + 2, h + 2)):
    raise gars.GarInputError(f"ext must be a contiguous float64 device tensor of shape ({h + 2}, {h + 2})")


def _attack_id(attack, direction):
  kind = _lib.ATTACK_LITTLE if attack == "little" else _lib.ATTACK_EMPIRE
  return kind | (_lib.ATTACK_DIRECTION if direction else 0)


def stack_stats_async(samples, scale=None, attack="empire", want_avg=True, direction=False):
  k, d, device = gars._validate(samples)
  lib = _lib.load()
  avg = torch.empty(d, dtype=torch.float32, device=device) if want_avg else None
  scaled = torch.empty(d, dtype=torch.float32, device=device) if scale is not None else None
  out3 = torch.empty(3, dtype=torch.float64, device=device)
  ws = gars._workspace(device, _lib.WS_STATS, k, d, "ws_stats")
  with torch.cuda.device(device):
    _lib.check(lib.bm_stack_stats(_lib.pointer_table(samples), k, d, _opt(avg), _opt(scaled),
                                  ctypes.c_float(scale if scale is not None else 0.0),
                                  _attack_id(attack, direction), _ptr(out3),
                                  _ptr(ws), gars._stream(device)), "bm_stack_stats")
  if scale is not None:
    return avg, out3, scaled
  return avg, out3


def compute_avg_dev_max(samples):
  if len(samples) == 0:
    return None, math.nan, math.nan, math.nan
  avg, out3 = stack_stats_async(samples)
  norm2, dev2, amax = out3.tolist()
  k = len(samples)
  norm_dev = math.sqrt(dev2 / (k - 1)) if k >= 2 else math.nan
  return avg, math.sqrt(norm2), norm_dev, amax


def study_dots(core, extra=()):
  core = list(core)
  extra = list(extra)
  nc, d, device = gars._validate(core)
  if extra:
    gars._validate(extra + [core[0]])
  lib = _lib.load()
  out = torch.empty(nc * nc + len(extra), dtype=torch.float64, device=device)
  ws = gars._workspace(device, _lib.WS_DOT, 1, d, "ws_dot")
  with torch.cuda.device(device):
    _lib.check(lib.bm_multi_dot(_lib.pointer_table(core), nc,
                                _lib.pointer_table(extra) if extra else None, len(extra), d, _ptr(out),
                                _ptr(ws), gars._stream(device)), "bm_multi_dot")
  return out[:nc * nc].view(nc, nc), out[nc * nc:]


_EVAL_OPS = {"trmean": _lib.OP_TRMEAN, "phocas": _lib.OP_PHOCAS, "meamed": _lib.OP_MEAMED, "median": _lib.OP_MEDIAN}


def colwise_eval_supported(rule, n):
  return rule in _EVAL_OPS and bool(_lib.load().bm_colwise_eval_supported(_EVAL_OPS[rule], n))


def colwise_eval(rule, honests, copies, f, h_avg, direction, t):
  honests = list(honests)
  h, d, device = gars._validate(honests)
  gars._validate([h_avg, direction] + honests[:1])
  lib = _lib.load()
  out = torch.empty(1, dtype=torch.float64, device=device)
  ws = gars._Scratch.get(device, "ws_eval", nbytes=int(lib.bm_colwise_eval_workspace_bytes()))
  with torch.cuda.device(device):
    if isinstance(t, torch.Tensor):
      _require_scalar_on(t, device, "colwise_eval: a tensor t must be a contiguous float64 tensor on the vectors' device")
      _lib.check(lib.bm_colwise_eval_tdev(_EVAL_OPS[rule], _lib.pointer_table(honests), h, copies, d, f, _ptr(h_avg),
                                          _ptr(direction), _ptr(t), _ptr(out), _ptr(ws), gars._stream(device)),
                 "bm_colwise_eval_tdev")
    else:
      _lib.check(lib.bm_colwise_eval(_EVAL_OPS[rule], _lib.pointer_table(honests), h, copies, d, f, _ptr(h_avg),
                                     _ptr(direction), float(t), _ptr(out), _ptr(ws), gars._stream(device)),
                 "bm_colwise_eval")
  return out


def sqdist2(a, b):
  _, d, device = gars._validate([a, b])
  lib = _lib.load()
  out = torch.empty(1, dtype=torch.float64, device=device)
  ws = gars._Scratch.get(device, "ws_eval", nbytes=int(lib.bm_colwise_eval_workspace_bytes()))
  with torch.cuda.device(device):
    _lib.check(lib.bm_sqdist2(_ptr(a), _ptr(b), d, _ptr(out), _ptr(ws), gars._stream(device)), "bm_sqdist2")
  return out


def bulyan_pass2_eval_supported(n, f, m, d=0):
  return d <= (1 << 29) and bool(_lib.load().bm_bulyan_pass2_eval_supported(int(n), int(f), int(m)))


def bulyan_pass2_eval(honests, copies, order, f, m, h_avg, direction, t):
  honests = list(honests)
  h, d, device = gars._validate(honests)
  gars._validate([h_avg, direction] + honests[:1])
  lib = _lib.load()
  out = torch.empty(1, dtype=torch.float64, device=device)
  ws = gars._Scratch.get(device, "ws_eval", nbytes=int(lib.bm_colwise_eval_workspace_bytes()))
  t_dev = None
  if isinstance(t, torch.Tensor):
    _require_scalar_on(t, device, "bulyan_pass2_eval: a tensor t must be a contiguous float64 tensor on the vectors' device")
    t_dev, t = t, 0.0
  with torch.cuda.device(device):
    _lib.check(lib.bm_bulyan_pass2_eval(_lib.pointer_table(honests), h, int(copies), _ptr(order), int(f), int(m), d,
                                        _ptr(h_avg), _ptr(direction), ctypes.c_float(float(t)), _opt(t_dev), _ptr(out),
                                        _ptr(ws), gars._stream(device)), "bm_bulyan_pass2_eval")
  return out


def order_pair_supported(h):
  return bool(_lib.load().bm_order_pair_supported(int(h)))


def order_pair(rows, il, ih):
  rows = list(rows)
  h, d, device = gars._validate(rows)
  lib = _lib.load()
  lo, hi = torch.empty_like(rows[0]), torch.empty_like(rows[0])
  with torch.cuda.device(device):
    _lib.check(lib.bm_order_pair(_lib.pointer_table(rows), h, d, int(il), int(ih), _ptr(lo), _ptr(hi),
                                 gars._stream(device)), "bm_order_pair")
  return lo, hi


class DeviceSearch:

  def __init__(self, device, evals, negative=False, start=0., delta=1., ratio=0.8):
    if not isinstance(evals, int) or evals < 1:
      _lib.check(_lib.EINVAL, "DeviceSearch (evals must be a positive integer)")
    self.device, self.evals, self.negative, self.shape = device, evals, bool(negative), (start, delta, ratio)
    self.state = torch.zeros(8, dtype=torch.float64, device=device)
    self.t = torch.zeros(1, dtype=torch.float64, device=device)
    self.out = torch.zeros(1 + 2 * evals, dtype=torch.float64, device=device)
    self.proposed = 0
    self._keep = None

  def _call(self, y, last):
    if y is not None and not (isinstance(y, torch.Tensor) and y.is_cuda and y.device == self.device
                              and y.dtype == torch.float64 and y.numel() >= 1):
      raise gars.GarInputError("DeviceSearch: the objective must be a float64 tensor on the search's device")
    lib = _lib.load()
    self._keep = y
    with torch.cuda.device(self.device):
      _lib.check(lib.bm_search_device_next(_ptr(self.state), _opt(y), 1 if self.negative else 0,
                                           1 if last else 0, *self.shape, _ptr(self.t) if not last else None,
                                           _ptr(self.out), gars._stream(self.device)), "bm_search_device_next")

  def next(self, y=None):
    if self.proposed >= self.evals or (y is None) != (self.proposed == 0):
      raise RuntimeError("DeviceSearch.next: one objective per candidate, `evals` candidates")
    self._call(y, False)
    self.proposed += 1
    return self.t

  def finish(self, y):
    if self.proposed != self.evals:
      raise RuntimeError("DeviceSearch.finish: the search has candidates left")
    self._call(y, True)
    return self.out


def study_stats(s_avg, h_avg, defense, byz, f_real, past_newest=None, curv=None, past_oldest=None, curv_mode=0, mu=0.0,
                oldest_weight=0.0, params=None, origin=None, attack_avg_out=None, update_momentum=None, update_mu=0.0,
                update_omd=0.0):
  vecs = [t for t in (s_avg, h_avg, defense, byz if f_real > 0 else None, past_newest if curv_mode >= 2 else None,
                      curv if curv_mode >= 1 else None, past_oldest if curv_mode == 3 else None, params, origin,
                      attack_avg_out, update_momentum) if t is not None]
  _, d, device = gars._validate(vecs)
  if (params is None) != (origin is None):
    raise gars.GarInputError("study_stats needs both params and origin, or neither")
  lib = _lib.load()
  out = torch.empty(_lib.STUDY_SLOTS, dtype=torch.float64, device=device)
  ws = gars._workspace(device, _lib.WS_STUDY, 1, d, "ws_study")
  with torch.cuda.device(device):
    _lib.check(lib.bm_study_stats_update(_ptr(s_avg), _ptr(h_avg), _ptr(defense), _opt(byz if f_real > 0 else None),
                                         int(f_real), _opt(attack_avg_out), _opt(past_newest), _opt(curv), _opt(past_oldest),
                                         int(curv_mode), ctypes.c_float(mu), ctypes.c_float(oldest_weight), _opt(params),
                                         _opt(origin), _opt(update_momentum), ctypes.c_float(update_mu),
                                         ctypes.c_float(update_omd), d, _ptr(out), _ptr(ws), gars._stream(device)),
               "bm_study_stats_update")
  if update_momentum is not None:
    gars.invalidate_rank_cache()
  return out


def row_sqnorms(gradients):
  n, d, device = gars._validate(gradients)
  lib = _lib.load()
  res = torch.empty(_lib.MAX_ROWS, dtype=torch.float64, device=device)
  ws = gars._workspace(device, _lib.WS_DOT, 1, d, "ws_dot")
  with torch.cuda.device(device):
    _lib.check(lib.bm_row_sqnorms(_lib.pointer_table(gradients), n, d, _ptr(res), _ptr(ws), gars._stream(device)),
               "bm_row_sqnorms")
  return res[:n]


def anticge_sum(gradients, f_decl, row_sq):
  h, d, device = gars._validate(gradients)
  if not 1 <= f_decl <= h:
    raise gars.GarInputError(f"anticge needs 1 <= f_decl <= {h} honest gradients, got f_decl = {f_decl}")
  if not (isinstance(row_sq, torch.Tensor) and row_sq.device == device and row_sq.dtype == torch.float64
          and row_sq.numel() >= h and row_sq.is_contiguous()):
    raise gars.GarInputError("anticge_sum: row_sq must be a contiguous float64 tensor of h squared norms on the gradients' device")
  lib = _lib.load()
  out = torch.empty(d, dtype=torch.float32, device=device)
  order = torch.empty(_lib.MAX_ROWS, dtype=torch.int32, device=device)
  scal = torch.empty(2, dtype=torch.float64, device=device)
  ws = gars._Scratch.get(device, "ws_anticge", nbytes=int(lib.bm_anticge_workspace_bytes(d)))
  with torch.cuda.device(device):
    _lib.check(lib.bm_anticge_sum(_lib.pointer_table(gradients), h, d, int(f_decl), _ptr(row_sq), _ptr(out), _ptr(order),
                                  _ptr(scal), _ptr(ws), gars._stream(device)), "bm_anticge_sum")
  return out, order, scal


def anticge_scale(vec, scal):
  _, d, device = gars._validate([vec])
  _require_scalar_on(scal, device, "anticge_scale: scal must be a contiguous float64 tensor on the vector's device")
  if scal.numel() < 2:
    raise gars.GarInputError("anticge_scale: scal must hold the two scalars anticge_sum left")
  lib = _lib.load()
  gars.invalidate_rank_cache()
  with torch.cuda.device(device):
    _lib.check(lib.bm_anticge_scale(_ptr(vec), d, _ptr(scal), gars._stream(device)), "bm_anticge_scale")
  return vec


def anticge_attack(grad_honests, f_decl, f_real, **kwargs):
  grad_honests = list(grad_honests)
  h, d, device = gars._validate(grad_honests)
  if f_real <= 0:
    return []
  if f_real > f_decl:
    return [torch.full_like(grad_honests[0], math.nan)] * f_real
  byz, _, scal = anticge_sum(grad_honests, f_decl, row_sqnorms(grad_honests).contiguous())
  return [anticge_scale(byz, scal)] * f_real


def attack_vector(kind, h_avg, factor=None, target=None, want_direction=False):
  if kind not in _lib.ATTACK_VECTOR_KINDS:
    raise gars.GarInputError(f"attack_vector: unknown kind {kind!r} (one of {sorted(_lib.ATTACK_VECTOR_KINDS)})")
  _, d, device = gars._validate([h_avg])
  shift = kind in ("shift_one", "shift_all")
  if want_direction and not shift:
    raise gars.GarInputError(f"attack_vector: kind {kind!r} has no direction vector to store")
  if kind != "nan" and factor is None:
    raise gars.GarInputError(f"attack_vector: kind {kind!r} needs a factor")
  target = -1 if target is None or kind != "shift_one" else int(target)
  if not -1 <= target < d:
    raise gars.GarInputError(f"attack_vector: target must be a coordinate within [0, {d}) or -1, got {target}")
  lib = _lib.load()
  out = torch.empty_like(h_avg)
  direction = torch.empty_like(h_avg) if want_direction else None
  with torch.cuda.device(device):
    if isinstance(factor, torch.Tensor):
      _require_scalar_on(factor, device, "attack_vector: a tensor factor must be a contiguous float64 tensor on the vector's device")
      host, dev = 0.0, _ptr(factor)
    else:
      host, dev = (0.0 if factor is None else float(factor)), None
    _lib.check(lib.bm_attack_vector(_lib.ATTACK_VECTOR_KINDS[kind], _ptr(h_avg), d, target, ctypes.c_float(host), dev,
                                    _ptr(out), _opt(direction), gars._stream(device)), "bm_attack_vector")
  return (out, direction) if want_direction else out


def _searched(grad_honests, avg, candidate, f_real, f_decl, defense, evals, kwargs):
  from . import linesearch
  if not callable(defense):
    raise gars.GarInputError(f"a searched attack needs the aggregation rule to defeat as `defense`, got {defense!r}")

  def scape(x):
    aggregated = defense(gradients=(grad_honests + [candidate(x)] * f_real), f=f_decl, model=kwargs.get("model"))
    return sqdist2(aggregated, avg).item()
  return linesearch.line_maximize(scape, evals=evals)[0]


def nan_attack(grad_honests, f_real, **kwargs):
  grad_honests = list(grad_honests)
  gars._validate(grad_honests)
  if f_real <= 0:
    return []
  return [attack_vector("nan", grad_honests[0])] * f_real


def bulyan_attack(grad_honests, f_real, f_decl=None, defense=None, factor=-16, negative=False, target_idx=-1, **kwargs):
  grad_honests = list(grad_honests)
  _, d, device = gars._validate(grad_honests)
  if f_real <= 0:
    return []
  if target_idx == "all":
    kind, target = "shift_all", None
  else:
    if not isinstance(target_idx, int) or isinstance(target_idx, bool):
      raise gars.GarInputError(f"expected an integer or \"all\" for 'target_idx', got {target_idx!r}")
    if not -d <= target_idx < d:
      raise IndexError(f"index {target_idx} is out of bounds for dimension 0 with size {d}")
    kind, target = "shift_one", target_idx % d
  avg = stack_stats_async(grad_honests)[0]
  if factor < 0:
    sign = -1.0 if negative else 1.0
    factor = _searched(grad_honests, avg, lambda x: attack_vector(kind, avg, sign * x, target), f_real, f_decl, defense,
                       math.ceil(-factor), kwargs)
  elif negative:
    factor = -factor
  return [attack_vector(kind, avg, factor, target)] * f_real


def empire_strict_attack(grad_honests, f_real, f_decl=None, defense=None, epsilon=1, **kwargs):
  grad_honests = list(grad_honests)
  gars._validate(grad_honests)
  if f_real <= 0:
    return []
  avg = stack_stats_async(grad_honests)[0]
  if epsilon < 0:
    epsilon = _searched(grad_honests, avg, lambda x: attack_vector("scale", avg, -x), f_real, f_decl, defense,
                        math.ceil(-epsilon), kwargs)
  return [attack_vector("scale", avg, -epsilon)] * f_real


def accept_count(order, count, h):
  if not (isinstance(order, torch.Tensor) and order.is_cuda and order.dtype == torch.int32 and order.dim() == 1
          and order.is_contiguous()):
    raise gars.GarInputError("accept_count: order must be a contiguous 1-D int32 tensor on a GPU")
  if not 0 <= count <= min(_lib.MAX_ROWS, order.numel()) or h < 0:
    raise gars.GarInputError(f"accept_count: count must be within 0..{min(_lib.MAX_ROWS, order.numel())} and h >= 0, "
                             f"got count = {count}, h = {h}")
  device = order.device
  out = torch.empty(1, dtype=torch.float64, device=device)
  with torch.cuda.device(device):
    _lib.check(_lib.load().bm_accept_count(_ptr(order), int(count), int(h), _ptr(out), gars._stream(device)),
               "bm_accept_count")
  return out


def multi_axpby(ys, xs, a, b):
  k, d, device = gars._validate(list(ys))
  gars._validate(list(xs) + [ys[0]])
  if len(xs) != k:
    raise gars.GarInputError("multi_axpby needs as many x as y vectors")
  lib = _lib.load()
  gars.invalidate_rank_cache()
  with torch.cuda.device(device):
    _lib.check(lib.bm_multi_axpby(_lib.pointer_table(ys), _lib.pointer_table(xs), k, d,
                                  ctypes.c_float(a), ctypes.c_float(b), gars._stream(device)),
               "bm_multi_axpby")


def momentum_stats(sampled, buffers, mu, one_minus_damp, clip_factors_dev=None, attack_scale=None, attack="empire",
                   direction=False):
  ks, d, device = gars._validate(list(sampled))
  h = gars._validate(list(buffers) + [sampled[0]])[0] - 1
  if h < 1 or ks < h:
    raise gars.GarInputError("momentum_stats needs 1 <= len(buffers) <= len(sampled)")
  lib = _lib.load()
  s_avg = torch.empty(d, dtype=torch.float32, device=device)
  h_avg = torch.empty(d, dtype=torch.float32, device=device)
  byz = torch.empty(d, dtype=torch.float32, device=device) if attack_scale is not None else None
  out6 = torch.empty(6, dtype=torch.float64, device=device)
  ws = gars._workspace(device, _lib.WS_STEP, 1, d, "ws_step")
  gars.invalidate_rank_cache()
  with torch.cuda.device(device):
    _lib.check(lib.bm_momentum_stats(
      _lib.pointer_table(sampled), ks, _lib.pointer_table(buffers), h, d, ctypes.c_float(mu),
      ctypes.c_float(one_minus_damp), _opt(clip_factors_dev), _ptr(s_avg), _ptr(h_avg), _opt(byz),
      ctypes.c_float(attack_scale if attack_scale is not None else 0.0),
      _attack_id(attack, direction), _ptr(out6), _ptr(ws),
      gars._stream(device)), "bm_momentum_stats")
  return s_avg, h_avg, byz, out6


def momentum_stats_colwise(sampled, buffers, mu, one_minus_damp, clip_factors_dev, attack_scale, attack, rule, f, n_byz):
  ks, d, device = gars._validate(list(sampled))
  h = gars._validate(list(buffers) + [sampled[0]])[0] - 1
  if h < 1 or ks < h or n_byz < 1:
    raise gars.GarInputError("momentum_stats_colwise needs 1 <= len(buffers) <= len(sampled) and n_byz >= 1")
  lib = _lib.load()
  s_avg, h_avg, byz, defense = (torch.empty(d, dtype=torch.float32, device=device) for _ in range(4))
  out6 = torch.empty(6, dtype=torch.float64, device=device)
  ws = gars._workspace(device, _lib.WS_STEP, 1, d, "ws_step")
  gars.invalidate_rank_cache()
  with torch.cuda.device(device):
    _lib.check(lib.bm_momentum_stats_colwise(
      _lib.pointer_table(sampled), ks, _lib.pointer_table(buffers), h, d, ctypes.c_float(mu),
      ctypes.c_float(one_minus_damp), _opt(clip_factors_dev),
      _ptr(s_avg), _ptr(h_avg), _ptr(byz), ctypes.c_float(attack_scale), _attack_id(attack, False),
      _EVAL_OPS[rule], int(f), int(n_byz), _ptr(defense), _ptr(out6), _ptr(ws), gars._stream(device)),
      "bm_momentum_stats_colwise")
  return s_avg, h_avg, byz, defense, out6


def momentum_stats_sqdist(sampled, buffers, mu, one_minus_damp, clip_factors_dev, attack_scale, attack, n_byz,
                          d_total=None):
  ks, d, device = gars._validate(list(sampled))
  h = gars._validate(list(buffers) + [sampled[0]])[0] - 1
  if h < 1 or ks < h or n_byz < 1 or h + n_byz > _lib.MAX_ROWS:
    raise gars.GarInputError("momentum_stats_sqdist needs 1 <= len(buffers) <= len(sampled), n_byz >= 1, at most 64 rows")
  n = h + n_byz
  lib = _lib.load()
  s_avg, h_avg, byz = (torch.empty(d, dtype=torch.float32, device=device) for _ in range(3))
  sq = torch.empty((n, n), dtype=torch.float64, device=device)
  out6 = torch.empty(6, dtype=torch.float64, device=device)
  ws = gars._workspace(device, _lib.WS_STEP, 1, d, "ws_step")
  ws_pair = gars._workspace(device, _lib.WS_PAIRWISE, n, d, "ws_pair")
  gars.invalidate_rank_cache()
  with torch.cuda.device(device):
    _lib.check(lib.bm_momentum_stats_sqdist(
      _lib.pointer_table(sampled), ks, _lib.pointer_table(buffers), h, d, d if d_total is None else int(d_total),
      ctypes.c_float(mu), ctypes.c_float(one_minus_damp), _opt(clip_factors_dev), _ptr(s_avg), _ptr(h_avg), _ptr(byz),
      ctypes.c_float(attack_scale), _attack_id(attack, False), int(n_byz), _ptr(sq), _ptr(out6), _ptr(ws), _ptr(ws_pair),
      gars._stream(device)), "bm_momentum_stats_sqdist")
  return s_avg, h_avg, byz, sq, out6


def stack_stats_colwise(rows, attack_scale, attack, rule, f, n_byz):
  k, d, device = gars._validate(list(rows))
  if n_byz < 1:
    raise gars.GarInputError("stack_stats_colwise needs n_byz >= 1")
  lib = _lib.load()
  avg, byz, defense = (torch.empty(d, dtype=torch.float32, device=device) for _ in range(3))
  out6 = torch.empty(6, dtype=torch.float64, device=device)
  ws = gars._workspace(device, _lib.WS_STEP, 1, d, "ws_step")
  with torch.cuda.device(device):
    _lib.check(lib.bm_stack_stats_colwise(_lib.pointer_table(rows), k, d, _ptr(avg), _ptr(byz),
                                          ctypes.c_float(attack_scale), _attack_id(attack, False), _EVAL_OPS[rule],
                                          int(f), int(n_byz), _ptr(defense), _ptr(out6), _ptr(ws),
                                          gars._stream(device)), "bm_stack_stats_colwise")
  return avg, byz, defense, out6


def stack_stats_sqdist(rows, attack_scale, attack, n_byz, d_total=None):
  k, d, device = gars._validate(list(rows))
  if n_byz < 1 or k + n_byz > _lib.MAX_ROWS:
    raise gars.GarInputError("stack_stats_sqdist needs n_byz >= 1 and at most 64 rows")
  n = k + n_byz
  lib = _lib.load()
  avg, byz = (torch.empty(d, dtype=torch.float32, device=device) for _ in range(2))
  sq = torch.empty((n, n), dtype=torch.float64, device=device)
  out6 = torch.empty(6, dtype=torch.float64, device=device)
  ws = gars._workspace(device, _lib.WS_STEP, 1, d, "ws_step")
  ws_pair = gars._workspace(device, _lib.WS_PAIRWISE, n, d, "ws_pair")
  with torch.cuda.device(device):
    _lib.check(lib.bm_stack_stats_sqdist(_lib.pointer_table(rows), k, d, d if d_total is None else int(d_total),
                                         _ptr(avg), _ptr(byz), ctypes.c_float(attack_scale), _attack_id(attack, False),
                                         int(n_byz), _ptr(sq), _ptr(out6), _ptr(ws), _ptr(ws_pair),
                                         gars._stream(device)), "bm_stack_stats_sqdist")
  return avg, byz, sq, out6


def multi_fma3(outs, ps, qs, a, b, p_scale_dev=None):
  outs, ps, qs = list(outs), list(ps), list(qs)
  k, d, device = gars._validate(outs)
  gars._validate(ps + [outs[0]])
  gars._validate(qs + [outs[0]])
  if len(ps) != k or len(qs) != k:
    raise gars.GarInputError("multi_fma3 needs as many p and q as out vectors")
  lib = _lib.load()
  gars.invalidate_rank_cache()
  scale = _opt(p_scale_dev)
  with torch.cuda.device(device):
    if isinstance(b, torch.Tensor):
      _require_scalar_on(b, device, "multi_fma3: a tensor b must be a contiguous float64 tensor on the vectors' device")
      _lib.check(lib.bm_multi_fma3_bdev(_lib.pointer_table(outs), _lib.pointer_table(ps), _lib.pointer_table(qs), k, d,
                                        ctypes.c_float(a), _ptr(b), scale, gars._stream(device)), "bm_multi_fma3_bdev")
    else:
      _lib.check(lib.bm_multi_fma3(_lib.pointer_table(outs), _lib.pointer_table(ps), _lib.pointer_table(qs), k, d,
                                   ctypes.c_float(a), ctypes.c_float(b), scale, gars._stream(device)), "bm_multi_fma3")


DEVICE_SEARCH_RULES = ("krum", "average")


def attack_search_device(ext, h, k, f, rule, evals=16, negative=False, m=None):
  if rule not in DEVICE_SEARCH_RULES:
    raise ValueError(f"no device form of the search for rule {rule!r}")
  _require_ext(ext, h)
  if not isinstance(evals, int) or evals < 1:
    _lib.check(_lib.EINVAL, "attack_search_device (evals must be a positive integer)")
  lib = _lib.load()
  extra = 24 * evals if os.environ.get("BM_SEARCH_TRACE", "") == "1" else 0
  out = torch.zeros(1 + 2 * evals + extra, dtype=torch.float64, device=ext.device) if extra else \
      torch.empty(1 + 2 * evals, dtype=torch.float64, device=ext.device)
  with torch.cuda.device(ext.device):
    _lib.check(lib.bm_attack_line_search_device(_ptr(ext), h, k, f, _lib.RULE_IDS[rule], m or 0, evals,
                                                1 if negative else 0, _ptr(out), gars._stream(ext.device)),
               "bm_attack_line_search_device")
  return out


def attack_ranking_device(ext, h, k, f, mode, t_dev, m=None):
  _require_ext(ext, h)
  _require_scalar_on(t_dev, ext.device, "attack_ranking_device: the factor must be a contiguous float64 tensor on the matrix's device")
  lib = _lib.load()
  order = torch.empty(_lib.MAX_ROWS, dtype=torch.int32, device=ext.device)
  mode_id = {"krum": _lib.RANK_KRUM, "bulyan": _lib.RANK_BULYAN}[mode]
  with torch.cuda.device(ext.device):
    _lib.check(lib.bm_attack_ranking_device(_ptr(ext), h, k, f, mode_id, m or 0, _ptr(t_dev), _ptr(order),
                                            gars._stream(ext.device)), "bm_attack_ranking_device")
  return order


def clip_factors_from_sq(sq, k, clip):
  lib = _lib.load()
  device = sq.device
  if not sq.is_contiguous():
    sq = sq.contiguous()
  factors = torch.empty(_lib.MAX_ROWS, dtype=torch.float32, device=device)
  with torch.cuda.device(device):
    _lib.check(lib.bm_clip_factors(_ptr(sq), k, ctypes.c_float(clip), _ptr(factors), gars._stream(device)),
               "bm_clip_factors")
  return factors


def clip_factors(gradients, clip):
  k, d, device = gars._validate(gradients)
  return clip_factors_from_sq(row_sqnorms(gradients), k, clip)


def multi_scale(ys, factors_dev):
  ys = list(ys)
  k, d, device = gars._validate(ys)
  lib = _lib.load()
  gars.invalidate_rank_cache()
  with torch.cuda.device(device):
    _lib.check(lib.bm_multi_scale(_lib.pointer_table(ys), k, d, _ptr(factors_dev), gars._stream(device)),
               "bm_multi_scale")


def clip_gradients(gradients, clip):
  factors = clip_factors(gradients, clip)
  multi_scale(gradients, factors)
  return factors


def l2_distance(a, b):
  return gars.pairwise_sqdist([a, b])[0, 1].sqrt()


def step_worker(comm, sampled, buffers, n, f_decl, f_real, rule, m, mu, one_minus_damp, clip, attack, attack_scale,
                nb_past, past_count, past_newest, curv, past_oldest, params=None, origin=None, d_total=None):
  ks, d, device = gars._validate(list(sampled))
  lib = _lib.load()
  new = lambda: torch.empty(d, dtype=torch.float32, device=device)
  defense, s_avg, h_avg = new(), new(), new()
  byz = new() if f_real > 0 else None
  stats = torch.empty(lib.bm_step_stats_count(), dtype=torch.float64, device=device)
  ws = gars._Scratch.get(device, "ws_stepcall", nbytes=int(lib.bm_step_workspace_bytes(n, d)))
  par = _lib.StepParams(n=n, f_decl=f_decl, f_real=f_real, ks=ks, rule=_lib.RULE_IDS[rule], m=m or 0,
                        attack_kind=_lib.ATTACK_LITTLE if attack == "little" else _lib.ATTACK_EMPIRE, nb_past=nb_past,
                        past_count=past_count, attack_scale=attack_scale, mu=mu, one_minus_damp=one_minus_damp,
                        clip=clip if clip is not None else 0.0,
                        oldest_weight=-(mu ** (nb_past - 1)) if nb_past > 0 else 0.0)
  gars.invalidate_rank_cache()
  with torch.cuda.device(device):
    _lib.check(lib.bm_step_worker(comm.handle if comm is not None else None, ctypes.byref(par),
                                  _lib.pointer_table(sampled), _lib.pointer_table(buffers), d,
                                  int(d_total) if d_total is not None else d, _ptr(defense),
                                  _ptr(s_avg), _ptr(h_avg), _opt(byz), None, _opt(past_newest), _opt(curv),
                                  _opt(past_oldest), _opt(params), _opt(origin), _ptr(stats), _ptr(ws),
                                  gars._stream(device)), "bm_step_worker")
  return defense, s_avg, h_avg, byz, stats
```

byzantinemomentum_amd/step.py:

```python

import collections
import math
from typing import NamedTuple, Optional

import torch

from . import _lib, linesearch

__all__ = ["AggregationStep"]

_RULES = ("krum", "bulyan", "median", "trmean", "phocas", "meamed", "aksel", "brute", "average", "cge")
_COLWISE = ("median", "trmean", "phocas", "meamed")
_DISTANCE = ("krum", "bulyan")
_ATTACKS = ("empire", "little", "anticge", "nan", "hidden", "empire-strict")
_VECTOR_ATTACKS = ("nan", "hidden", "empire-strict")
MAX_PAST = 4096


class StepPlan(NamedTuple):
  only_m: bool
  analytic: bool
  first_pass: str
  search: Optional[str]
  device_cursor: bool
  single_call: bool
  capabilities: frozenset
  accept: Optional[str] = None


_StudyRecord = collections.namedtuple("_StudyRecord",
                                      "s2 sd smax h2 hd hmax a2 ad amax d2 dmax l2 gram ex0 ex1 prev_s2 accept")
_ACCEPT_COUNTED = ("krum", "brute", "aksel", "cge")


class AggregationStep:
  def __init__(self, nb_workers, nb_decl_byz, nb_real_byz, gar="krum", gar_args=None, momentum=0.99,
               dampening=0.99, momentum_at="worker", attack="empire", attack_factor=1.1, nb_past=25,
               gradient_clip=None, aggregator=None, single_call=True, attack_evals=None, attack_negative=False,
               line_search="auto", attack_args=None):
    if gar not in _RULES:
      raise ValueError(f"unknown aggregation rule {gar!r}")
    if momentum_at not in ("worker", "server", "update"):
      raise ValueError(f"momentum_at must be 'worker', 'server' or 'update', got {momentum_at!r}")
    if attack not in _ATTACKS:
      hint = "; the reference's `bulyan` attack is \"hidden\" here (bulyan names a rule)" if attack == "bulyan" else ""
      raise ValueError(f"unknown attack {attack!r} (empire, little, hidden: factor, use a negative one for negative:True; "
                       f"empire-strict: epsilon; anticge, nan: no factor){hint}")
    if attack_evals is not None and (not isinstance(attack_evals, int) or attack_evals < 1):
      raise ValueError(f"attack_evals must be a positive number of evaluations, got {attack_evals!r}")
    if attack == "anticge":
      if attack_evals is not None:
        raise ValueError("the anticge attack has no factor to search: attack_evals must be None")
      if nb_real_byz >= 1 and not 1 <= nb_decl_byz <= nb_workers - nb_real_byz:
        raise ValueError(f"the anticge attack needs 1 <= nb_decl_byz <= {nb_workers - nb_real_byz} honest workers "
                         f"(attacks/anticge.py:67-68 indexes the sorted norms at h - f_decl), got {nb_decl_byz}")
    if attack_args is not None and (attack != "hidden" or not isinstance(attack_args, dict)
                                    or set(attack_args) - {"target_idx"}):
      raise ValueError(f"attack_args holds {{'target_idx': int | 'all'}} for the hidden attack and nothing else, "
                       f"got {attack_args!r} with attack {attack!r}")
    target_idx = (attack_args or {}).get("target_idx", -1)
    if attack == "hidden" and target_idx != "all" and (not isinstance(target_idx, int) or isinstance(target_idx, bool)):
      raise ValueError(f"target_idx must be an integer or \"all\" (attacks/identical.py:121-124), got {target_idx!r}")
    if attack == "nan" and attack_evals is not None:
      raise ValueError("the nan attack has no factor to search: attack_evals must be None")
    if attack == "empire-strict":
      if attack_negative:
        raise ValueError("the empire-strict attack has no `negative` (attacks/empire.py:29): attack_negative must be False")
      if attack_evals is None and (not isinstance(attack_factor, int) or isinstance(attack_factor, bool) or attack_factor < 1):
        raise ValueError(f"the empire-strict attack takes a positive integer epsilon as attack_factor "
                         f"(attacks/empire.py:82), got {attack_factor!r}")
    if line_search not in ("auto", "host", "generic"):
      raise ValueError(f"line_search must be 'auto', 'host' or 'generic', got {line_search!r}")
    if not 0 <= nb_past <= MAX_PAST:
      raise ValueError(f"nb_past must be within 0..{MAX_PAST}")
    if aggregator is None:
      from .sharded import ShardedAggregator
      aggregator = ShardedAggregator()
    self.agg = aggregator
    self.ops = aggregator.backend
    self.n = nb_workers
    self.f_decl = nb_decl_byz
    self.f_real = nb_real_byz
    self.h = nb_workers - nb_real_byz
    self.gar = gar
    self.gar_args = dict(gar_args or {})
    self.mu = momentum
    self.damp = dampening
    self.momentum_at = momentum_at
    self.attack = attack
    self.target_idx = target_idx
    self.factor = attack_factor
    self.clip = gradient_clip
    self.attack_evals = attack_evals
    self.attack_negative = bool(attack_negative)
    self.line_search = line_search
    self._factor_now = attack_factor
    self._search_now = None
    self.last_byzantine = None
    self.buffers = None
    self.server_momentum = None
    self.pasts = collections.deque(maxlen=max(nb_past, 1))
    self.nb_past = nb_past
    self._prev_s2 = None
    self._curv = None
    self._pending = None
    self._update = None
    self._prev_stats = None
    self.plan = self._make_plan(single_call)
    self.single_call = self.plan.single_call

  def _make_plan(self, single_call):
    caps = frozenset(getattr(self.ops, "capabilities", ()))
    gar, k, fixed = self.gar, self.f_real, self.attack_evals is None
    only_m = not (set(self.gar_args) - {"m"})
    analytic = self.line_search in ("auto", "host")
    stem = {"worker": "momentum_stats_", "update": "stack_stats_"}.get(self.momentum_at)
    behind = self.attack == "anticge" or self.attack in _VECTOR_ATTACKS
    strict = self.attack == "empire-strict"
    if not fixed and self.attack != "hidden":
      first_pass = "direction"
    elif behind:
      first_pass = "plain"
    elif stem and k >= 1 and not self.gar_args and gar in _COLWISE and stem + "colwise" in caps:
      first_pass = "rule"
    elif stem and k >= 1 and only_m and gar in _DISTANCE and stem + "sqdist" in caps:
      first_pass = "sqdist"
    else:
      first_pass = "plain"
    small = self.h + 2 <= 64
    device_cursor = self.line_search == "auto" and "device_search" in caps and gar != "brute"
    if fixed:
      search, device_cursor = None, False
    elif analytic and gar in linesearch.ANALYTIC_RULES and small and only_m:
      device_cursor = self.line_search == "auto" and gar in getattr(self.ops, "device_search_rules", ()) and not strict
      search = "scalar_device" if device_cursor else "scalar_host"
    elif analytic and gar == "bulyan" and k >= 1 and small and only_m:
      search, device_cursor = "bulyan", device_cursor and "attack_ranking_device" in caps
    elif analytic and gar == "median" and k >= 1:
      search = "median"
    elif analytic and gar in _COLWISE and k >= 1 and not self.gar_args and "colwise_eval" in caps:
      search = "colwise_eval"
    else:
      search = "generic"
    single = bool(single_call and fixed and not behind and self.momentum_at == "worker" and "step_worker" in caps
                  and gar in _DISTANCE + _COLWISE and only_m and (not self.agg.collective or self.agg.native is not None))
    accept = "count" if gar in _ACCEPT_COUNTED else ("average" if gar == "average" else None)
    return StepPlan(only_m, analytic, first_pass, search, device_cursor, single, caps, accept)


  @property
  def last_factor(self):
    if isinstance(self._factor_now, torch.Tensor):
      self._settle_search()
    return self._factor_now

  @last_factor.setter
  def last_factor(self, value):
    self._factor_now = value

  @property
  def last_search(self):
    if isinstance(self._search_now, torch.Tensor):
      self._settle_search()
    return self._search_now

  @last_search.setter
  def last_search(self, value):
    self._search_now = value

  def _settle_search(self):
    values = self._fetch(self._search_now).tolist()
    self._factor_now = values[0]
    self._search_now = [(values[1 + 2 * i], values[2 + 2 * i]) for i in range((len(values) - 1) // 2)]

  @staticmethod
  def _new_rows(count, like, zero=False):
    return [torch.zeros_like(like) if zero else torch.empty_like(like) for _ in range(count)]

  def _aggregate(self, gradients):
    agg, f = self.agg, self.f_decl
    if self.gar == "median":
      return agg.median(gradients)
    if self.gar == "average":
      return agg.average(gradients)
    if self.gar == "brute":
      return agg.brute(gradients, f, check=True, **self.gar_args)
    return getattr(agg, self.gar)(gradients, f, **self.gar_args)

  def _fetch(self, matrix):
    if not matrix.is_cuda:
      return matrix.contiguous()
    key = (tuple(matrix.shape), matrix.dtype)
    if getattr(self, "_pinned", None) is None or self._pinned[0] != key:
      self._pinned = (key, torch.empty(matrix.shape, dtype=matrix.dtype, pin_memory=True))
    host = self._pinned[1]
    host.copy_(matrix, non_blocking=True)
    torch.cuda.current_stream(matrix.device).synchronize()
    return host

  def _search_factor(self, honests, h_avg, direction):
    plan = self.plan
    if plan.search in ("scalar_device", "scalar_host"):
      return self._search_scalar(honests, h_avg, direction)
    on_device = plan.device_cursor and h_avg.is_cuda
    form = {"bulyan": self._bulyan_objective, "median": self._median_objective,
            "colwise_eval": self._colwise_objective, "generic": self._generic_objective}[plan.search]
    return self._drive(form(honests, h_avg, direction, on_device), h_avg, on_device,
                       shift=1.0 if self.attack == "empire-strict" else 0.0)

  def _drive(self, evaluate, h_avg, on_device, shift=0.0):
    def objective(t):
      sq = evaluate(t + shift if shift else t)
      self.agg.all_reduce_sum(sq)
      return sq

    if on_device:
      cursor = self.ops.device_search(h_avg.device, self.attack_evals, self.attack_negative)
      y = None
      for _ in range(self.attack_evals):
        y = objective(cursor.next(y))
      found = self.last_search = cursor.finish(y)
      return found
    factor, self.last_search = linesearch.line_maximize(
      lambda x: objective(-x if self.attack_negative else x).item(), evals=self.attack_evals)
    return factor

  def _unit_sqdist(self, honests, h_avg, direction):
    unit = torch.empty_like(h_avg)
    self.ops.multi_fma3([unit], [h_avg], [direction], 1.0, 1.0)
    return self.agg.global_sqdist(list(honests) + [h_avg, unit])

  def _search_scalar(self, honests, h_avg, direction):
    sq = self._unit_sqdist(honests, h_avg, direction)
    args = dict(evals=self.attack_evals, negative=self.attack_negative, m=self.gar_args.get("m"))
    if self.plan.search == "scalar_device":
      found = self.last_search = self.ops.attack_search_device(sq, self.h, self.f_real, self.f_decl, self.gar, **args)
      return found
    ext = self._fetch(sq)
    if self.attack == "empire-strict":
      factor, self.last_search = linesearch.line_maximize(
        lambda x: linesearch.attack_objective(ext, self.h, self.f_real, self.f_decl, self.gar, 1.0 + x, args["m"])[0],
        evals=self.attack_evals)
      return factor
    factor, self.last_search = linesearch.attack_line_search(ext, self.h, self.f_real, self.f_decl, self.gar, **args)
    return factor

  def _written_objective(self, rule, h_avg, direction):
    ops = self.ops

    def evaluate(t):
      cand = torch.empty_like(h_avg)
      ops.multi_fma3([cand], [h_avg], [direction], 1.0, t)
      out = rule(cand, t)
      if "sqdist2" in self.plan.capabilities:
        return ops.sqdist2(out, h_avg)
      return ops.pairwise_sqdist([out, h_avg])[0, 1].reshape(1)
    return evaluate

  def _generic_objective(self, honests, h_avg, direction, on_device=False):
    return self._written_objective(lambda cand, t: self._aggregate(list(honests) + [cand] * self.f_real), h_avg, direction)

  def _colwise_objective(self, honests, h_avg, direction, on_device=False):
    ops, k = self.ops, self.f_real
    if not ops.colwise_eval_supported(self.gar, self.h + k):
      return self._generic_objective(honests, h_avg, direction)
    return lambda t: ops.colwise_eval(self.gar, honests, k, self.f_decl, h_avg, direction, t)

  def _median_objective(self, honests, h_avg, direction, on_device=False):
    ops, agg, h, k = self.ops, self.agg, self.h, self.f_real
    n, caps = h + k, self.plan.capabilities
    if "order_pair" in caps and ops.order_pair_supported(h):
      lo, hi = ops.order_pair(honests, (n - 1) // 2 - k, (n - 1) // 2)
    else:
      lo = agg.median(list(honests) + [torch.full_like(h_avg, -math.inf)] * k)
      hi = agg.median(list(honests) + [torch.full_like(h_avg, math.inf)] * k)
    if "colwise_eval" in caps:
      whole = not self.gar_args and ops.colwise_eval_supported("median", n)
      if ops.colwise_eval_supported("median", 3):
        return lambda t: ops.colwise_eval("median", [lo, hi], 1, 0, h_avg, direction, t)
      if whole:
        return lambda t: ops.colwise_eval("median", honests, k, self.f_decl, h_avg, direction, t)
    return self._written_objective(lambda cand, t: agg.median([cand, lo, hi]), h_avg, direction)

  def _bulyan_objective(self, honests, h_avg, direction, on_device):
    ops, h, k, f = self.ops, self.h, self.f_real, self.f_decl
    n = h + k
    m = self.gar_args.get("m") or n - f - 2
    sq_dev = self._unit_sqdist(honests, h_avg, direction)
    ext = None if on_device else self._fetch(sq_dev)

    def ranking(t):
      if on_device:
        return ops.attack_ranking_device(sq_dev, h, k, f, "bulyan", t, m)
      order = linesearch.attack_ranking(ext, h, k, f, "bulyan", t, m)
      return ops.index_tensor(order + [0] * (64 - n), h_avg)

    if "bulyan_pass2_eval" in self.plan.capabilities and ops.bulyan_pass2_eval_supported(n, f, m, h_avg.shape[0]):
      return lambda t: ops.bulyan_pass2_eval(honests, k, ranking(t), f, m, h_avg, direction, t)
    return self._written_objective(lambda cand, t: ops.bulyan_pass2(list(honests) + [cand] * k, ranking(t), f, m),
                                   h_avg, direction)

  def nesterov_lookahead(self, params, lr, worker=None):
    mom = (self.buffers[worker] if self.buffers is not None else None) if worker is not None else self.server_momentum
    if mom is not None:
      self.ops.multi_fma3([params], [params], [mom], 1.0, -(self.mu * lr))
    return params

  def run(self, grad_sampleds, params=None, origin=None):
    ops, agg, h = self.ops, self.agg, self.h
    sampled = list(grad_sampleds)
    if getattr(grad_sampleds, "d_total", None) is not None:
      from .sharded import Shards
      sampled = Shards(sampled, d_total=grad_sampleds.d_total)
    ks = len(sampled)
    if ks < h:
      raise ValueError(f"{ks} sampled gradients for {h} honest workers")
    omd = 1.0 - self.damp
    if self.single_call:
      return self._run_single_call(sampled, ks, omd, params, origin)
    factors = None
    if self.clip is not None:
      sq = ops.row_sqnorms(sampled)
      agg.all_reduce_sum(sq)
      factors = ops.clip_factors_from_sq(sq, ks, self.clip)
    fused_defense, fused_sq = None, None
    first_pass = self.plan.first_pass
    searched = self.attack_evals is not None
    with_direction = first_pass == "direction"
    anticge = self.attack == "anticge"
    vector, strict = self.attack in _VECTOR_ATTACKS, self.attack == "empire-strict"
    kind = "empire" if strict else self.attack
    scale = None if anticge or (vector and not with_direction) else (1.0 if searched else self.factor)
    if self.momentum_at == "worker":
      if self.buffers is None:
        self.buffers = self._new_rows(h, sampled[0], zero=True)
      if first_pass == "rule":
        s_avg, h_avg, byz, fused_defense, out6 = ops.momentum_stats_colwise(
          sampled, self.buffers, self.mu, omd, factors, self.factor, self.attack, self.gar, self.f_decl, self.f_real)
      elif first_pass == "sqdist":
        s_avg, h_avg, byz, fused_sq, out6 = ops.momentum_stats_sqdist(
          sampled, self.buffers, self.mu, omd, factors, self.factor, self.attack, self.f_real,
          d_total=agg._total_of(sampled))
      else:
        s_avg, h_avg, byz, out6 = ops.momentum_stats(sampled, self.buffers, self.mu, omd, factors, scale, kind,
                                                     direction=with_direction)
      honests = self.buffers
      s_out3, h_out3 = out6[:3], out6[3:]
    else:
      if factors is not None:
        ops.multi_scale(sampled, factors)
      if self.momentum_at == "server":
        mom = self.server_momentum if self.server_momentum is not None else torch.zeros_like(sampled[0])
        honests = self._new_rows(h, sampled[0])
        ops.multi_fma3(honests, sampled[:h], [mom] * h, omd, self.mu)
      else:
        honests = sampled[:h]
      if ks != h and first_pass in ("rule", "sqdist"):
        first_pass = "plain"
      if first_pass == "rule":
        h_avg, byz, fused_defense, o6 = ops.stack_stats_colwise(honests, self.factor, self.attack, self.gar, self.f_decl,
                                                                self.f_real)
        h_out3 = o6[3:]
      elif first_pass == "sqdist":
        h_avg, byz, fused_sq, o6 = ops.stack_stats_sqdist(honests, self.factor, self.attack, self.f_real,
                                                          d_total=agg._total_of(sampled))
        h_out3 = o6[3:]
      else:
        h_avg, h_out3, *byz = ops.stack_stats(honests, scale=scale, attack=kind, direction=with_direction)
        byz = byz[0] if byz else None
      if self.momentum_at == "update" and ks == h:
        s_avg, s_out3 = h_avg, h_out3
      else:
        s_avg, s_out3 = ops.stack_stats(sampled)
    if anticge and self.f_real > 0:
      byz = agg.anticge(honests, self.f_decl, self.f_real)[0]
    if vector and self.f_real > 0:
      if self.attack == "nan":
        byz = agg.attack_vector("nan", h_avg)
      elif self.attack == "hidden":
        where = dict(target_idx=self.target_idx, d_total=agg._total_of(sampled)) if self.target_idx != "all" else {}
        made = agg.attack_vector("shift_all" if self.target_idx == "all" else "shift_one", h_avg,
                                 1.0 if searched else self.factor, want_direction=searched, **where)
        byz = made[1] if searched else made
      elif not searched:
        byz = agg.attack_vector("scale", h_avg, -self.factor)
    if searched and self.f_real > 0:
      direction = byz
      factor = self._search_factor(honests, h_avg, direction)
      self.last_factor = factor
      if strict:
        byz = agg.attack_vector("scale", h_avg, -factor[:1] if isinstance(factor, torch.Tensor) else -factor)
      else:
        byz = torch.empty_like(h_avg)
        ops.multi_fma3([byz], [h_avg], [direction], 1.0, factor)
    attacks = [byz] * self.f_real
    self.last_byzantine = byz if self.f_real > 0 else None
    if fused_defense is not None:
      defense = fused_defense
    elif fused_sq is not None:
      defense = agg.rule_from_sq(self.gar, honests + attacks, fused_sq, self.f_decl, self.gar_args.get("m"))
    else:
      defense = self._aggregate(honests + attacks)
    accept, accept_of = self._accept_count() if self.plan.accept == "count" else (None, None)
    if self.momentum_at == "server":
      self.server_momentum = defense
      self._update = defense
    elif self.momentum_at == "update":
      if self.server_momentum is None:
        self.server_momentum = torch.zeros_like(defense)
      self._update = self.server_momentum
    else:
      self._update = defense
    count = len(self.pasts) if self.nb_past > 0 else 0
    mode = 0
    if self.nb_past > 0:
      if self._curv is None:
        self._curv = torch.empty_like(s_avg)
      mode = 1 if count == 0 else (3 if count == self.nb_past else 2)
    has_l2 = params is not None and origin is not None
    study = ops.study_stats(s_avg, h_avg, defense, byz if self.f_real > 0 else None, self.f_real,
                            past_newest=self.pasts[0] if count > 0 else None, curv=self._curv,
                            past_oldest=self.pasts[-1] if mode == 3 else None, curv_mode=mode, mu=self.mu,
                            oldest_weight=-(self.mu ** (self.nb_past - 1)) if self.nb_past > 0 else 0.0,
                            params=params if has_l2 else None, origin=origin if has_l2 else None,
                            **(dict(update_momentum=self.server_momentum, update_mu=self.mu, update_omd=omd)
                               if self.momentum_at == "update" else {}))
    self._pending = dict(s=s_out3, h=h_out3, study=study, npast=2 if count > 0 else 0,
                         prev_s2=self._prev_s2 if count > 0 else None, has_l2=has_l2, ks=ks, floats=None, accept=accept,
                         accept_of=accept_of)
    if self.nb_past > 0:
      self.pasts.appendleft(s_avg)
      self._prev_s2 = s_out3[:1]
    return defense

  def _accept_count(self):
    order, count = self.agg.last_selection
    if "accept_count" in self.plan.capabilities:
      return self.ops.accept_count(order, count, self.h), count
    return (order[:count] >= self.h).sum().to(torch.float64).reshape(1), count

  def _run_single_call(self, sampled, ks, omd, params, origin):
    h = self.h
    if self.buffers is None:
      self.buffers = self._new_rows(h, sampled[0], zero=True)
    count = len(self.pasts) if self.nb_past > 0 else 0
    if self.nb_past > 0 and self._curv is None:
      self._curv = torch.empty_like(sampled[0])
    full = count == self.nb_past and count > 0
    defense, s_avg, h_avg, byz, stats = self.ops.step_worker(
      self.agg.native, sampled, self.buffers, self.n, self.f_decl, self.f_real, self.gar, self.gar_args.get("m"),
      self.mu, omd, self.clip, self.attack, self.factor, self.nb_past, count,
      self.pasts[0] if count > 0 else None, self._curv, self.pasts[-1] if full else None, params, origin,
      d_total=self.agg._total_of(sampled))
    self._update = defense
    self.last_byzantine = byz
    self._pending = dict(packed=stats, prev=self._prev_stats if count > 0 else None, npast=2 if count > 0 else 0,
                         has_l2=params is not None and origin is not None, ks=ks,
                         floats=None,
                         accept_of=self.gar_args.get("m") or self.n - self.f_decl - 2)
    if self.nb_past > 0:
      self.pasts.appendleft(s_avg)
      self._prev_stats = stats
    return defense

  def update_gradient(self):
    return self._update


  def _exchange(self, pend):
    s3, h3, st, prev = pend["s"], pend["h"], pend["study"], pend["prev_s2"]
    last = [prev] if prev is not None else []
    acc = [pend["accept"]] if pend["accept"] is not None else []
    if not self.agg.collective:
      flat = torch.cat([s3, h3, st] + last + acc).tolist()
      s3, h3, st, rest = flat[0:3], flat[3:6], flat[6:6 + _lib.STUDY_SLOTS], flat[6 + _lib.STUDY_SLOTS:]
      last, acc = rest[:len(last)], rest[len(last):]
      sums = s3[_lib.OUT3_SUMS] + h3[_lib.OUT3_SUMS] + st[_lib.STUDY_SUMS] + st[_lib.STUDY_L2] + last
      maxes = s3[_lib.OUT3_MAX] + h3[_lib.OUT3_MAX] + st[_lib.STUDY_MAXES] + acc
    else:
      sums, maxes = self.agg.exchange(
        torch.cat([s3[_lib.OUT3_SUMS], h3[_lib.OUT3_SUMS], st[_lib.STUDY_SUMS], st[_lib.STUDY_L2]] + last),
        torch.cat([s3[_lib.OUT3_MAX], h3[_lib.OUT3_MAX], st[_lib.STUDY_MAXES]] + acc))
      ns = int(sums.numel())
      flat = torch.cat([sums, maxes]).tolist()
      sums, maxes = flat[:ns], flat[ns:]
    s2, sd, h2, hd = sums[0:4]
    st = sums[4:24]
    gram, (ex0, ex1), (a2, ad) = st[_lib.STUDY_GRAM], st[_lib.STUDY_EX], st[_lib.STUDY_ATTACK]
    smax, hmax, amax, dmax = maxes[:4]
    return _StudyRecord(s2, sd, smax, h2, hd, hmax, a2, ad, amax, gram[4 * 2 + 2], dmax, sums[24], gram, ex0, ex1,
                        sums[25] if prev is not None else math.nan, maxes[4] if acc else math.nan)

  @staticmethod
  def _unpack(pend):
    vec = pend["packed"] if pend["prev"] is None else torch.cat([pend["packed"], pend["prev"][:1]])
    v = vec.tolist()
    L = _lib
    return _StudyRecord(v[L.STEP_S2], v[L.STEP_SD], v[L.STEP_SMAX], v[L.STEP_H2], v[L.STEP_HD], v[L.STEP_HMAX],
                        v[L.STEP_A2], v[L.STEP_AD], v[L.STEP_AMAX], v[L.STEP_D2], v[L.STEP_DMAX], v[L.STEP_L2],
                        v[L.STEP_GRAM], v[L.STEP_EX.start], v[L.STEP_EX.start + 1],
                        v[len(pend["packed"])] if pend["prev"] is not None else math.nan, v[L.STEP_ACCEPT])

  def _study_floats(self, rec, pend):
    nan = math.nan
    att, k_s, k_h, k_a = self.f_real > 0, pend["ks"], self.h, self.f_real
    g = rec.gram

    def dev(x, k):
      return math.sqrt(x / (k - 1)) if k >= 2 else nan

    def cos(i, j):
      if not att and 3 in (i, j):
        return nan
      return g[4 * i + j] / math.sqrt(g[5 * i]) / math.sqrt(g[5 * j])

    past = pend["npast"] > 0
    if self.plan.accept == "count":
      accept = int(rec.accept) / pend["accept_of"]
    else:
      accept = self.f_real / self.n if self.plan.accept == "average" else nan
    return {
      "l2_origin": math.sqrt(rec.l2) if pend["has_l2"] else nan,
      "sampled_norm_avg": math.sqrt(rec.s2), "sampled_norm_dev": dev(rec.sd, k_s), "sampled_norm_max": rec.smax,
      "honest_norm_avg": math.sqrt(rec.h2), "honest_norm_dev": dev(rec.hd, k_h), "honest_norm_max": rec.hmax,
      "attack_norm_avg": math.sqrt(rec.a2) if att else nan, "attack_norm_dev": dev(rec.ad, k_a) if att else nan,
      "attack_norm_max": rec.amax if att else nan,
      "defense_norm_avg": math.sqrt(rec.d2), "defense_norm_max": rec.dmax,
      "cosin_splhon": cos(0, 1), "cosin_spldef": cos(0, 2), "cosin_hondef": cos(1, 2),
      "cosin_splatt": cos(0, 3), "cosin_honatt": cos(1, 3), "cosin_attdef": cos(3, 2),
      "cosin_sampled": rec.ex0 / math.sqrt(rec.s2) / math.sqrt(rec.prev_s2) if past else nan,
      "curv_sampled": self.mu * rec.ex1 if past else nan,
      "accept_ratio": accept,
    }

  def floats(self):
    pend = self._pending
    if pend is None:
      raise RuntimeError("floats() needs a run() first")
    if pend["floats"] is None:
      if self.gar == "brute":
        self.agg.check_brute()
      pend["floats"] = self._study_floats(self._unpack(pend) if "packed" in pend else self._exchange(pend), pend)
    return pend["floats"]
```

include/bm_gar.h:

```cpp
#ifndef BM_GAR_H
#define BM_GAR_H

#include <stdint.h>

#ifdef __cplusplus
extern "C" {
#endif

#define BM_MAX_ROWS 64
#define BM_EINVAL   (-100000)
#define BM_ENOCOMM  (-100001)
#define BM_ECOMM    (-100002)

enum bm_colwise_op {
  BM_OP_MEDIAN = 0,
  BM_OP_TRMEAN = 1,
  BM_OP_PHOCAS = 2,
  BM_OP_MEAMED = 3
};

int bm_abi_version(void);
int bm_tuning_set(const char* name, int value);

const char* bm_error_string(int code);

int bm_colwise(int op, const float* const* rows, int n, int64_t d, int f,
               float* out, void* stream);

enum bm_ws_kind {
  BM_WS_PAIRWISE = 0,
  BM_WS_AKSEL    = 1,
  BM_WS_STATS    = 2,
  BM_WS_DOT      = 3,
  BM_WS_STEP     = 4,
  BM_WS_STUDY    = 5
};
int64_t bm_workspace_bytes(int kind, int n, int64_t d);

int bm_pairwise_sqdist(const float* const* rows, int n, int64_t d,
                       double* sq_nxn, void* ws, void* stream);

int bm_pairwise_sqdist_shard(const float* const* rows, int n, int64_t d, int64_t d_total,
                             double* sq_nxn, void* ws, void* stream);

enum bm_rank_mode { BM_RANK_KRUM = 0, BM_RANK_BULYAN = 1 };
int bm_krum_rank(const double* sq_nxn, int n, int f, int m, int mode,
                 int32_t* order_out, double* scores_out, void* stream);

int bm_pairwise_rank(const float* const* rows, int n, int64_t d, int64_t d_total, int f, int m, int mode,
                     double* sq_nxn, int32_t* order_out, double* scores_out, void* ws, void* stream);

int bm_selected_mean(const float* const* rows, int n, const int32_t* idx, int m,
                     int64_t d, float* out, void* stream);

int bm_bulyan_pass2(const float* const* rows, int n, const int32_t* order, int f, int m,
                    int64_t d, float* out, void* stream);

int bm_aksel_pass1(const float* const* rows, int n, int64_t d, float* median_out,
                   double* sq_out, void* ws, void* stream);

enum bm_attack_kind { BM_ATTACK_EMPIRE = 0, BM_ATTACK_LITTLE = 1,
                      BM_ATTACK_DIRECTION = 16 };
int bm_stack_stats(const float* const* rows, int k, int64_t d, float* avg_out,
                   float* scaled_out, float scale, int attack_kind, double* out3, void* ws,
                   void* stream);

int bm_multi_dot(const float* const* core, int nc, const float* const* extra, int ne,
                 int64_t d, double* out, void* ws, void* stream);

#define BM_STUDY_SLOTS 32
int bm_study_stats(const float* sampled_avg, const float* honest_avg, const float* defense, const float* byz,
                   int f_real, float* attack_avg_out, const float* past_newest, float* curv,
                   const float* past_oldest, int curv_mode, float mu, float oldest_weight, const float* params,
                   const float* origin, int64_t d, double* out, void* ws, void* stream);
int bm_study_stats_update(const float* sampled_avg, const float* honest_avg, const float* defense, const float* byz,
                          int f_real, float* attack_avg_out, const float* past_newest, float* curv,
                          const float* past_oldest, int curv_mode, float mu, float oldest_weight, const float* params,
                          const float* origin, float* update_momentum, float momentum_mu, float one_minus_damp,
                          int64_t d, double* out, void* ws, void* stream);

int bm_row_sqnorms(const float* const* rows, int k, int64_t d, double* sq_out, void* ws, void* stream);

int bm_stable_argsort(const double* keys, int n, int32_t* order_out, void* stream);

int64_t bm_anticge_workspace_bytes(int64_t d);
int bm_anticge_sum(const float* const* rows, int h, int64_t d, int f_decl, const double* row_sq, float* sum_out,
                   int32_t* order_out, double* scal_out, void* ws, void* stream);
int bm_anticge_scale(float* vec, int64_t d, const double* scal, void* stream);

enum bm_attack_vector_kind { BM_AV_NAN = 0, BM_AV_SHIFT_ONE = 1, BM_AV_SHIFT_ALL = 2, BM_AV_SCALE = 3 };
int bm_attack_vector(int kind, const float* avg, int64_t d, int64_t target, float factor, const double* factor_dev,
                     float* out, float* direction_out, void* stream);

int bm_multi_axpby(float* const* y, const float* const* x, int k, int64_t d,
                   float a, float b, void* stream);

int bm_momentum_stats(const float* const* sampled, int ks, float* const* buffers, int h, int64_t d,
                      float mu, float one_minus_damp, const float* clip_factors, float* sampled_avg,
                      float* honest_avg, float* byz_out, float scale, int attack_kind, double* out6,
                      void* ws, void* stream);

int bm_momentum_stats_colwise(const float* const* sampled, int ks, float* const* buffers, int h, int64_t d,
                              float mu, float one_minus_damp, const float* clip_factors, float* sampled_avg,
                              float* honest_avg, float* byz_out, float scale, int attack_kind, int rule_op,
                              int rule_f, int n_byz, float* defense_out, double* out6, void* ws, void* stream);

int bm_momentum_stats_sqdist(const float* const* sampled, int ks, float* const* buffers, int h, int64_t d,
                             int64_t d_total, float mu, float one_minus_damp, const float* clip_factors,
                             float* sampled_avg, float* honest_avg, float* byz_out, float scale, int attack_kind,
                             int n_byz, double* sq_nxn, double* out6, void* ws, void* ws_pair, void* stream);

int bm_stack_stats_colwise(const float* const* rows, int k, int64_t d, float* avg_out, float* byz_out, float scale,
                           int attack_kind, int rule_op, int rule_f, int n_byz, float* defense_out, double* out6,
                           void* ws, void* stream);
int bm_stack_stats_sqdist(const float* const* rows, int k, int64_t d, int64_t d_total, float* avg_out, float* byz_out,
                          float scale, int attack_kind, int n_byz, double* sq_nxn, double* out6, void* ws,
                          void* ws_pair, void* stream);

int bm_multi_fma3(float* const* out, const float* const* p, const float* const* q, int k, int64_t d,
                  float a, float b, const float* p_scale, void* stream);
int bm_multi_fma3_bdev(float* const* out, const float* const* p, const float* const* q, int k, int64_t d,
                       float a, const double* b_dev, const float* p_scale, void* stream);

int bm_clip_factors(const double* row_sq, int k, float clip, float* factors_out, void* stream);
int bm_multi_scale(float* const* y, int k, int64_t d, const float* factors, void* stream);

int bm_brute_select(const double* dist_nxn, int n, int f, int32_t* sel_out);
int bm_brute_select_device(const double* sq_nxn, int n, int f, int32_t* sel_out, int32_t* status, void* stream);

typedef struct bm_comm bm_comm;

int bm_comm_available(void);
int bm_comm_unique_id(void* id128);
int bm_comm_init(bm_comm** out, int nranks, int rank, const void* id128);
int bm_comm_destroy(bm_comm* comm);
int bm_comm_size(const bm_comm* comm);

int bm_allreduce_sum_f64(bm_comm* comm, double* buf, int64_t count, void* stream);
int bm_allgather_f32(bm_comm* comm, const float* mine, float* all, int64_t count_per_rank, void* stream);

int64_t bm_sharded_workspace_bytes(int n, int64_t d_local);
int bm_sharded_krum(bm_comm* comm, const float* const* rows, int n, int64_t d_local, int64_t d_total, int f, int m,
                    float* out_local, int32_t* order_out, void* ws, void* stream);
int bm_sharded_bulyan(bm_comm* comm, const float* const* rows, int n, int64_t d_local, int64_t d_total, int f, int m,
                      float* out_local, int32_t* order_out, void* ws, void* stream);

double* bm_sharded_sq_slot(void* ws);
void* bm_sharded_pair_workspace(void* ws);
int32_t* bm_sharded_order_slot(void* ws);
int bm_sharded_rule_from_sq(bm_comm* comm, int rule, const float* const* rows, int n, int64_t d_local, int f, int m,
                            float* out_local, int32_t* order_out, void* ws, void* stream);

enum bm_step_rule { BM_RULE_KRUM = 0, BM_RULE_BULYAN = 1, BM_RULE_MEDIAN = 2, BM_RULE_TRMEAN = 3,
                    BM_RULE_PHOCAS = 4, BM_RULE_MEAMED = 5,
                    BM_RULE_BRUTE = 6, BM_RULE_AVERAGE = 7  };
typedef struct bm_step_params {
  int32_t n, f_decl, f_real;
  int32_t ks;
  int32_t rule;
  int32_t m;
  int32_t attack_kind;
  int32_t nb_past;
  int32_t past_count;
  float attack_scale;
  float mu, one_minus_damp;
  float clip;
  float oldest_weight;
} bm_step_params;
int bm_step_stats_count(void);
int64_t bm_step_workspace_bytes(int n, int64_t d_local);
int bm_step_worker(bm_comm* comm, const bm_step_params* p, const float* const* sampled, float* const* buffers,
                   int64_t d, int64_t d_total , float* defense_out,
                   float* sampled_avg_out, float* honest_avg_out, float* byz_out,
                   float* attack_avg_out, const float* past_newest, float* curv, const float* past_oldest,
                   const float* params, const float* origin, double* stats_out, void* ws, void* stream);

int bm_accept_count(const int32_t* order, int count, int h, double* out, void* stream);

int bm_colwise_eval_supported(int op, int n);
int64_t bm_colwise_eval_workspace_bytes(void);
int bm_colwise_eval(int op, const float* const* honests, int h, int copies, int64_t d, int f, const float* avg,
                    const float* dir, float t, double* out, void* ws, void* stream);
int bm_colwise_eval_tdev(int op, const float* const* honests, int h, int copies, int64_t d, int f, const float* avg,
                         const float* dir, const double* t_dev, double* out, void* ws, void* stream);

typedef struct bm_search {
  double best_x, best_y;
  double probe;
  double step, ratio;
  int32_t phase;
  int32_t evaluations;
  int32_t awaiting;
  int32_t reserved;
} bm_search;
int bm_search_begin(bm_search* c, double start, double delta, double ratio);
int bm_search_propose(bm_search* c, double* x_out);
int bm_search_report(bm_search* c, double y);
int bm_attack_objective(const double* ext, int h, int k, int f, int rule, int m, double t, double* y_out,
                        int32_t* sel_out, int32_t* count_out);
int bm_attack_line_search(const double* ext, int h, int k, int f, int rule, int m, int evals, int negative,
                          double* factor_out, double* trace_out);
int bm_attack_line_search_device(const double* ext, int h, int k, int f, int rule, int m, int evals, int negative,
                                 double* out, void* stream);
int bm_sqdist2(const float* a, const float* b, int64_t d, double* out, void* ws, void* stream);
int bm_attack_ranking_device(const double* ext, int h, int k, int f, int mode, int m, const double* t_dev,
                             int32_t* order_out, void* stream);
int bm_bulyan_pass2_eval_supported(int n, int f, int m);
int bm_bulyan_pass2_eval(const float* const* honests, int h, int copies, const int32_t* order, int f, int m, int64_t d,
                         const float* avg, const float* dir, float t, const double* t_dev, double* out, void* ws,
                         void* stream);
int bm_order_pair_supported(int h);
int bm_order_pair(const float* const* rows, int h, int64_t d, int il, int ih, float* lo, float* hi, void* stream);
int bm_search_device_next(void* state, const double* y, int negative, int last, double start, double delta, double ratio,
                          double* t_out, double* out, void* stream);
int bm_attack_ranking(const double* ext, int h, int k, int f, int mode, int m, double t, int32_t* order_out);

#ifdef __cplusplus
}
#endif
#endif
```

Baseline: 5163.

## Speculatively evaluate line-search tree of candidates in one fused colwise pass

Replaces the sequential attack line search, which runs one colwise evaluation per probe, with a speculative binary tree of probes. Every possible outcome path over the next few steps (up to depth 4, 15 nodes) is evaluated in a single kernel that loads and sorts each column once and scores all candidate factors against it. A device kernel then resolves which path the sequential search would have taken. This cuts the number of full memory passes and launches by about the tree depth, at the cost of wasted compute on probes that are never used and higher register pressure.

```diff
diff --git a/byzantinemomentum_amd/_lib.py b/byzantinemomentum_amd/_lib.py
--- a/byzantinemomentum_amd/_lib.py
+++ b/byzantinemomentum_amd/_lib.py
@@ -34,6 +34,7 @@
 SIGNATURES = {
   "bm_abi_version": (ctypes.c_int, []),
   "bm_tuning_set": (ctypes.c_int, [ctypes.c_char_p, ctypes.c_int]),
+  "bm_search_tree_depth": (ctypes.c_int, []),
   "bm_error_string": (ctypes.c_char_p, [ctypes.c_int]),
   "bm_colwise": (ctypes.c_int, [ctypes.c_int, _c_float_pp, ctypes.c_int, ctypes.c_int64, ctypes.c_int,
                                 ctypes.c_void_p, ctypes.c_void_p]),
@@ -128,6 +129,12 @@
   "bm_colwise_eval_tdev": (ctypes.c_int, [ctypes.c_int, _c_float_pp, ctypes.c_int, ctypes.c_int, ctypes.c_int64,
                                           ctypes.c_int, ctypes.c_void_p, ctypes.c_void_p, ctypes.c_void_p, ctypes.c_void_p,
                                           ctypes.c_void_p, ctypes.c_void_p]),
+  "bm_colwise_tree_eval_supported": (ctypes.c_int, [ctypes.c_int, ctypes.c_int, ctypes.c_int]),
+  "bm_colwise_tree_eval_max": (ctypes.c_int, [ctypes.c_int, ctypes.c_int, ctypes.c_int]),
+  "bm_colwise_tree_eval_workspace_bytes": (ctypes.c_int64, []),
+  "bm_colwise_tree_eval": (ctypes.c_int, [ctypes.c_int, _c_float_pp, ctypes.c_int, ctypes.c_int, ctypes.c_int64, ctypes.c_int,
+                                          ctypes.c_void_p, ctypes.c_void_p, ctypes.c_void_p, ctypes.c_void_p, ctypes.c_int,
+                                          ctypes.c_void_p, ctypes.c_void_p, ctypes.c_void_p]),
   "bm_sqdist2": (ctypes.c_int, [ctypes.c_void_p, ctypes.c_void_p, ctypes.c_int64, ctypes.c_void_p, ctypes.c_void_p,
                                 ctypes.c_void_p]),
   "bm_attack_ranking_device": (ctypes.c_int, [ctypes.c_void_p, ctypes.c_int, ctypes.c_int, ctypes.c_int, ctypes.c_int, ctypes.c_int,
@@ -142,6 +149,9 @@
   "bm_search_device_next": (ctypes.c_int, [ctypes.c_void_p, ctypes.c_void_p, ctypes.c_int, ctypes.c_int, ctypes.c_double,
                                            ctypes.c_double, ctypes.c_double, ctypes.c_void_p, ctypes.c_void_p,
                                            ctypes.c_void_p]),
+  "bm_search_device_tree_next": (ctypes.c_int, [ctypes.c_void_p, ctypes.c_void_p, ctypes.c_int, ctypes.c_double, ctypes.c_int,
+                                                ctypes.c_int, ctypes.c_double, ctypes.c_double, ctypes.c_double,
+                                                ctypes.c_void_p, ctypes.c_void_p, ctypes.c_void_p]),
   "bm_pairwise_rank": (ctypes.c_int, [_c_float_pp, ctypes.c_int, ctypes.c_int64, ctypes.c_int64, ctypes.c_int, ctypes.c_int,
                                       ctypes.c_int, ctypes.c_void_p, ctypes.c_void_p, ctypes.c_void_p, ctypes.c_void_p,
                                       ctypes.c_void_p]),
@@ -158,6 +168,8 @@
   "bm_search_begin": (ctypes.c_int, [ctypes.c_void_p, ctypes.c_double, ctypes.c_double, ctypes.c_double]),
   "bm_search_propose": (ctypes.c_int, [ctypes.c_void_p, ctypes.c_void_p]),
   "bm_search_report": (ctypes.c_int, [ctypes.c_void_p, ctypes.c_double]),
+  "bm_search_tree_emit": (ctypes.c_int, [ctypes.c_void_p, ctypes.c_int, ctypes.c_void_p]),
+  "bm_search_tree_resolve": (ctypes.c_int, [ctypes.c_void_p, ctypes.c_int, ctypes.c_void_p, ctypes.c_void_p]),
   "bm_attack_objective": (ctypes.c_int, [ctypes.c_void_p, ctypes.c_int, ctypes.c_int, ctypes.c_int, ctypes.c_int,
                                          ctypes.c_int, ctypes.c_double, ctypes.c_void_p, ctypes.c_void_p,
                                          ctypes.c_void_p]),
diff --git a/byzantinemomentum_amd/csrc/api.cpp b/byzantinemomentum_amd/csrc/api.cpp
--- a/byzantinemomentum_amd/csrc/api.cpp
+++ b/byzantinemomentum_amd/csrc/api.cpp
@@ -22,7 +22,8 @@
                            env_int("BM_PAIR_PLANES", 0), env_int("BM_PAIR_DITHER", 0), env_double("BM_PAIR_TAU", 2e-3),
                            env_int("BM_STUDY_BURST", 8), env_int("BM_STEP_STAGGER_US", 0),
                            env_int("BM_GRAM_STEADY", 1), env_int("BM_BULYAN_SHORT", 1),
-                           env_int("BM_PAIR_LOAD_NT", 1), env_int("BM_RANK_ALGO", 0), env_int("BM_COL_WIDE", 1), env_int("BM_BRUTE_BUDGET", 0)};
+                           env_int("BM_PAIR_LOAD_NT", 1), env_int("BM_RANK_ALGO", 0), env_int("BM_COL_WIDE", 1),
+                           env_int("BM_SEARCH_TREE", 3), env_int("BM_BRUTE_BUDGET", 0)};
   return t;
 }
 const Tuning& tuning() { return tuning_mutable(); }
@@ -40,13 +41,19 @@
       {"BM_PAIR_DITHER", &t.pair_dither}, {"BM_STUDY_BURST", &t.study_burst},
       {"BM_STEP_STAGGER_US", &t.step_stagger_us}, {"BM_GRAM_STEADY", &t.gram_steady},
       {"BM_BULYAN_SHORT", &t.bulyan_short}, {"BM_PAIR_LOAD_NT", &t.pair_load_nt},
-      {"BM_RANK_ALGO", &t.rank_algo}, {"BM_COL_WIDE", &t.col_wide}, {"BM_BRUTE_BUDGET", &t.brute_budget}};
+      {"BM_RANK_ALGO", &t.rank_algo}, {"BM_COL_WIDE", &t.col_wide}, {"BM_SEARCH_TREE", &t.search_tree},
+      {"BM_BRUTE_BUDGET", &t.brute_budget}};
   for (const auto& k : knobs)
     if (strcmp(name, k.key) == 0) {
       *k.slot = value;
       return 0;
     }
   return BM_EINVAL;
+}
+
+extern "C" int bm_search_tree_depth(void) {
+  const int depth = bm::tuning().search_tree;
+  return depth < 1 ? 1 : (depth > 4 ? 4 : depth);
 }
 
 extern "C" const char* bm_error_string(int code) {
diff --git a/byzantinemomentum_amd/csrc/bm_common.h b/byzantinemomentum_amd/csrc/bm_common.h
--- a/byzantinemomentum_amd/csrc/bm_common.h
+++ b/byzantinemomentum_amd/csrc/bm_common.h
@@ -240,6 +240,7 @@
   int pair_load_nt;
   int rank_algo;
   int col_wide;
+  int search_tree;
   int brute_budget;
 };
 const Tuning& tuning();
diff --git a/byzantinemomentum_amd/csrc/linesearch.cpp b/byzantinemomentum_amd/csrc/linesearch.cpp
--- a/byzantinemomentum_amd/csrc/linesearch.cpp
+++ b/byzantinemomentum_amd/csrc/linesearch.cpp
@@ -142,6 +142,18 @@
   if (c == nullptr || !c->awaiting) return BM_EINVAL;
   cursor_report(c, y);
   c->awaiting = 0;
+  return 0;
+}
+
+extern "C" int bm_search_tree_emit(const bm_search* c, int depth, double* xs_out) {
+  if (c == nullptr || xs_out == nullptr || c->awaiting || depth < 1 || depth > kSearchTreeMaxDepth) return BM_EINVAL;
+  for (int i = 0; i < search_tree_nodes(depth); ++i) xs_out[i] = search_tree_node(c, i);
+  return 0;
+}
+
+extern "C" int bm_search_tree_resolve(bm_search* c, int depth, const double* ys, double* trace_out) {
+  if (c == nullptr || ys == nullptr || c->awaiting || depth < 1 || depth > kSearchTreeMaxDepth) return BM_EINVAL;
+  search_tree_resolve(c, depth, ys, trace_out);
   return 0;
 }
 
diff --git a/byzantinemomentum_amd/csrc/search_core.h b/byzantinemomentum_amd/csrc/search_core.h
--- a/byzantinemomentum_amd/csrc/search_core.h
+++ b/byzantinemomentum_amd/csrc/search_core.h
@@ -59,6 +59,65 @@
   ++c->evaluations;
 }
 
+constexpr int kSearchTreeMaxDepth = 4;
+constexpr int kSearchTreeMaxNodes = (1 << kSearchTreeMaxDepth) - 1;
+__host__ __device__ inline int search_tree_nodes(int depth) { return (1 << depth) - 1; }
+__host__ __device__ inline int search_tree_depth(int depth, int evals, int done) {
+  const int left = evals - done;
+  depth = depth > kSearchTreeMaxDepth ? kSearchTreeMaxDepth : depth;
+  depth = depth < left ? depth : left;
+  return depth < 0 ? 0 : depth;
+}
+
+__host__ __device__ inline void cursor_assume(bm_search* c, bool better) {
+  better = better || (c->phase == kSearchFirst);
+  if (better) c->best_x = c->probe;
+  switch (c->phase) {
+    case kSearchFirst:
+      c->phase = kSearchGrow;
+      break;
+    case kSearchGrow:
+      if (better) {
+        c->step *= 2.0;
+      } else {
+        c->step *= c->ratio;
+        c->phase = kSearchShrink;
+      }
+      break;
+    default:
+      c->step *= c->ratio;
+  }
+  ++c->evaluations;
+}
+
+__host__ __device__ inline double search_tree_node(const bm_search* c, int node) {
+  bm_search cur = *c;
+  const int j = node + 1;
+  int level = 0;
+  while ((j >> (level + 1)) != 0) ++level;
+  for (int l = level - 1; l >= 0; --l) {
+    cursor_propose(&cur);
+    cursor_assume(&cur, ((j >> l) & 1) != 0);
+  }
+  cursor_propose(&cur);
+  return cur.probe;
+}
+
+__host__ __device__ inline void search_tree_resolve(bm_search* c, int depth, const double* ys, double* trace) {
+  int node = 0;
+  for (int l = 0; l < depth; ++l) {
+    cursor_propose(c);
+    const double y = ys[node];
+    const bool better = (c->phase == kSearchFirst) || (y > c->best_y);
+    if (trace != nullptr) {
+      trace[2 * l] = c->probe;
+      trace[2 * l + 1] = y;
+    }
+    cursor_report(c, y);
+    node = 2 * node + (better ? 2 : 1);
+  }
+}
+
 __host__ __device__ inline double attack_w(double a_i, double c, double ext_i_att) { return 0.5 * (a_i + c - ext_i_att); }
 __host__ __device__ inline double attack_uu(double a_i, double a_j, double ext_ij, bool same) {
   return same ? a_i : 0.5 * (a_i + a_j - ext_ij);
diff --git a/byzantinemomentum_amd/csrc/search_device.hip b/byzantinemomentum_amd/csrc/search_device.hip
--- a/byzantinemomentum_amd/csrc/search_device.hip
+++ b/byzantinemomentum_amd/csrc/search_device.hip
@@ -290,6 +290,48 @@
   *state = cur;
 }
 
+__global__ __launch_bounds__(64) void search_tree_kernel(bm_search* __restrict__ state, const double* __restrict__ ys,
+                                                         int negative, double shift, int depth, int evals, double start,
+                                                         double delta, double ratio, double* __restrict__ t_out,
+                                                         double* __restrict__ out) {
+  __shared__ bm_search shared;
+  const int lane = threadIdx.x;
+  if (lane == 0) {
+    bm_search cur;
+    if (ys == nullptr) {
+      cursor_begin(&cur, start, delta, ratio);
+    } else {
+      cur = *state;
+      const int done = cur.evaluations;
+      search_tree_resolve(&cur, search_tree_depth(depth, evals, done), ys, out + 1 + 2 * done);
+    }
+    if (cur.evaluations >= evals) out[0] = cur.best_x;
+    *state = cur;
+    shared = cur;
+  }
+  __syncthreads();
+  const int next = search_tree_depth(depth, evals, shared.evaluations);
+  if (next > 0 && lane < search_tree_nodes(next)) {
+    const double x = search_tree_node(&shared, lane);
+    const double t = negative ? -x : x;
+    t_out[lane] = shift != 0.0 ? t + shift : t;
+  }
+}
+
+}
+
+extern "C" int bm_search_device_tree_next(void* state, const double* ys, int negative, double shift, int depth, int evals,
+                                          double start, double delta, double ratio, double* t_out, double* out,
+                                          void* stream) {
+  using namespace bm;
+  if (state == nullptr || out == nullptr || t_out == nullptr || depth < 1 || depth > kSearchTreeMaxDepth || evals < 1)
+    return BM_EINVAL;
+  if (ys == nullptr && (!(start >= 0.0) || !(delta > 0.0) || !(ratio > 0.5 && ratio < 1.0))) return BM_EINVAL;
+  hipLaunchKernelGGL(search_tree_kernel, dim3(1), dim3(64), 0, static_cast<hipStream_t>(stream),
+                     static_cast<bm_search*>(state), ys, negative ? 1 : 0, shift, depth, evals, start, delta, ratio, t_out,
+                     out);
+  BM_LAUNCH_CHECK();
+  return 0;
 }
 
 extern "C" int bm_search_device_next(void* state, const double* y, int negative, int last, double start, double delta,
diff --git a/byzantinemomentum_amd/csrc/search_tree.h b/byzantinemomentum_amd/csrc/search_tree.h
--- /dev/null
+++ b/byzantinemomentum_amd/csrc/search_tree.h
@@ -0,0 +1,195 @@
+#pragma once
+#include "colwise_kernels.h"
+#include "search_core.h"
+
+namespace bm {
+
+constexpr int kTreeCandStride = 2 * kEvalMaxBlocks;
+static_assert(kEvalCaps.sets() <= kTreeCandStride, "evaluate-only partials exceed their stride");
+
+struct TreeFactors {
+  float t[kSearchTreeMaxNodes];
+};
+
+template <int H, int K, int OP, int VEC, int C>
+__global__ __launch_bounds__(kColBlock) void colwise_tree_eval_kernel(RowTable rows, const float* __restrict__ avg,
+                                                                      const float* __restrict__ dir, TreeFactors t_host,
+                                                                      const double* __restrict__ t_dev, int count,
+                                                                      int64_t nvec, double* __restrict__ partial) {
+  constexpr int N = H + K, F = K;
+  constexpr int kKeep = (OP == BM_OP_TRMEAN) ? (N - 2 * F) : (N - F);
+  constexpr float kInvKeep = 1.0f / (float)kKeep;
+  const float kInf = __builtin_inff();
+  const float kNaN = __builtin_nanf("");
+  float t[C];
+#pragma unroll
+  for (int q = 0; q < C; ++q) {
+    t[q] = t_dev != nullptr ? (float)t_dev[q < count ? q : count - 1] : t_host.t[q];
+  }
+  __shared__ double red[kColBlock / 64];
+  float acc[C];
+  double wide[C];
+#pragma unroll
+  for (int q = 0; q < C; ++q) {
+    acc[q] = 0.0f;
+    wide[q] = 0.0;
+  }
+  int since = 0;
+  const int64_t stride = (int64_t)gridDim.x * kColBlock;
+  for (int64_t v = (int64_t)blockIdx.x * kColBlock + threadIdx.x; v < nvec; v += stride) {
+    const int64_t j = v * VEC;
+    float hs[VEC][H];
+    float a[VEC], dr[VEC];
+    load_stream<VEC>(avg + j, a);
+    load_stream<VEC>(dir + j, dr);
+    int zero;
+    asm volatile("s_mov_b32 %0, 0" : "=s"(zero));
+#pragma unroll
+    for (int i = 0; i < H; ++i) {
+      float tmp[VEC];
+      load_stream<VEC>(rows.p[i + zero] + j, tmp);
+#pragma unroll
+      for (int c = 0; c < VEC; ++c) hs[c][i] = tmp[c];
+    }
+#pragma unroll
+    for (int c = 0; c < VEC; ++c) {
+      bool honest_nan = false;
+#pragma unroll
+      for (int i = 0; i < H; ++i) honest_nan |= (hs[c][i] != hs[c][i]);
+      int honest_nans = 0;
+      if (__builtin_amdgcn_ballot_w64(honest_nan) != 0ull) {
+#pragma unroll
+        for (int i = 0; i < H; ++i) {
+          const bool isn = (hs[c][i] != hs[c][i]);
+          honest_nans += isn ? 1 : 0;
+          hs[c][i] = isn ? kInf : hs[c][i];
+        }
+      }
+      sort_network<H>(hs[c]);
+#pragma unroll
+      for (int q = 0; q < C; ++q) {
+        {
+          const float cand = __builtin_fmaf(t[q], dr[c], 1.0f * a[c]);
+          const bool cand_nan = (cand != cand);
+          const float b = cand_nan ? kInf : cand;
+          const int nan_count = honest_nans + (cand_nan ? K : 0);
+          float x[N];
+#pragma unroll
+          for (int r = 0; r < N; ++r) {
+            const float below = (r - K >= 0) ? hs[c][r - K < 0 ? 0 : r - K] : -kInf;
+            const float above = (r < H) ? hs[c][r < H ? r : 0] : kInf;
+            x[r] = __builtin_amdgcn_fmed3f(below, b, above);
+          }
+          float tsum = 0.0f;
+          if constexpr (OP == BM_OP_TRMEAN || OP == BM_OP_PHOCAS) tsum = trimmed_sum<N>(x, F);
+          float res;
+          if constexpr (OP == BM_OP_TRMEAN) {
+            const float r = div_small_int(tsum, (float)(N - 2 * F), kInvKeep);
+            res = (nan_count > F) ? kNaN : r;
+          } else {
+            float ctr;
+            if constexpr (OP == BM_OP_PHOCAS) {
+              ctr = div_small_int(tsum, (float)(N - 2 * F), 1.0f / (float)(N - 2 * F));
+              if (nan_count > F) ctr = kNaN;
+            } else {
+              ctr = (honest_nan || cand_nan) ? kNaN : x[(N - 1) / 2];
+            }
+            const float wsum = closest_sum<N>(x, F, ctr);
+            const float r = div_small_int(wsum, (float)(N - F), kInvKeep);
+            res = (ctr != ctr || nan_count > F) ? kNaN : r;
+          }
+          const float df = res - a[c];
+          acc[q] = __builtin_fmaf(df, df, acc[q]);
+        }
+      }
+    }
+    if (++since == 16) {
+#pragma unroll
+      for (int q = 0; q < C; ++q) {
+        wide[q] += (double)acc[q];
+        acc[q] = 0.0f;
+      }
+      since = 0;
+    }
+  }
+#pragma unroll
+  for (int q = 0; q < C; ++q) {
+    {
+      const double r = block_reduce_sum<kColBlock>(wide[q] + (double)acc[q], red);
+      if (threadIdx.x == 0) partial[(int64_t)q * kTreeCandStride + blockIdx.x] = r;
+    }
+  }
+}
+
+template <int THREADS>
+__global__ __launch_bounds__(THREADS) void tree_finish_kernel(const double* __restrict__ partial, int nparts,
+                                                              double* __restrict__ out) {
+  __shared__ double red[THREADS / 64];
+  const double* const mine = partial + (int64_t)blockIdx.x * kTreeCandStride;
+  double tot = 0.0;
+  for (int b = threadIdx.x; b < nparts; b += THREADS) tot += mine[b];
+  const double r = block_reduce_sum<THREADS>(tot, red);
+  if (threadIdx.x == 0) out[blockIdx.x] = r;
+}
+
+template <int H, int K, int OP, int C>
+static int launch_tree_eval_width(const float* const* rows, int64_t d, const float* avg, const float* dir,
+                                  const TreeFactors& t, const double* t_dev, int count, double* out, double* partial,
+                                  hipStream_t s) {
+  constexpr int kMaxVec = (H + K <= 28) ? 4 : 2;
+  RowTable tab{};
+  for (int i = 0; i < H; ++i) tab.p[i] = rows[i];
+  const int vec = Alignment().of(rows, H).of(avg).of(dir).vec();
+  int nparts = 0;
+  const int rc = for_body_and_tail<kMaxVec>(Tail::kOwnLaunch, vec, d, kColBlock, kEvalCaps, [&](auto width, const Span& sp) {
+    hipLaunchKernelGGL((colwise_tree_eval_kernel<H, K, OP, decltype(width)::value, C>), dim3(sp.grid), dim3(kColBlock), 0, s,
+                       tab.advanced(sp.first), advanced(avg, sp.first), advanced(dir, sp.first), t, t_dev, count, sp.count,
+                       partial + sp.part);
+    BM_LAUNCH_CHECK();
+    return 0;
+  }, &nparts);
+  if (rc != 0) return rc;
+  hipLaunchKernelGGL(tree_finish_kernel<kEvalFinishThreads>, dim3(count), dim3(kEvalFinishThreads), 0, s, partial, nparts, out);
+  BM_LAUNCH_CHECK();
+  return 0;
+}
+
+template <int H, int K, int OP>
+constexpr int tree_max_candidates() {
+  return (OP != BM_OP_TRMEAN && H == 27 && K == 24) ? 7 : kSearchTreeMaxNodes;
+}
+
+template <int H, int K, int OP>
+static int launch_tree_eval(const float* const* rows, int64_t d, const float* avg, const float* dir, const TreeFactors& t,
+                            const double* t_dev, int count, double* out, double* partial, hipStream_t s) {
+  if (count <= 1) return launch_tree_eval_width<H, K, OP, 1>(rows, d, avg, dir, t, t_dev, count, out, partial, s);
+  if (count <= 3) return launch_tree_eval_width<H, K, OP, 3>(rows, d, avg, dir, t, t_dev, count, out, partial, s);
+  if (count <= 7) return launch_tree_eval_width<H, K, OP, 7>(rows, d, avg, dir, t, t_dev, count, out, partial, s);
+  if constexpr (tree_max_candidates<H, K, OP>() >= kSearchTreeMaxNodes)
+    return launch_tree_eval_width<H, K, OP, kSearchTreeMaxNodes>(rows, d, avg, dir, t, t_dev, count, out, partial, s);
+  return BM_EINVAL;
+}
+
+template <int OP>
+static int launch_tree_eval_shape(int n, int k, const float* const* rows, int64_t d, const float* avg, const float* dir,
+                                  const TreeFactors& t, const double* t_dev, int count, double* out, double* partial,
+                                  hipStream_t s) {
+#define BM_TREE_SHAPE(NN, KK) \
+  if (n == (NN) && k == (KK)) return launch_tree_eval<(NN) - (KK), (KK), OP>(rows, d, avg, dir, t, t_dev, count, out, partial, s);
+  BM_TREE_SHAPE(11, 2) BM_TREE_SHAPE(25, 5) BM_TREE_SHAPE(25, 11) BM_TREE_SHAPE(51, 12) BM_TREE_SHAPE(51, 24)
+#undef BM_TREE_SHAPE
+  return BM_EINVAL;
+}
+
+int tree_eval_phocas(int n, int k, const float* const* rows, int64_t d, const float* avg, const float* dir,
+                     const TreeFactors& t, const double* t_dev, int count, double* out, double* partial, hipStream_t s);
+int tree_eval_meamed(int n, int k, const float* const* rows, int64_t d, const float* avg, const float* dir,
+                     const TreeFactors& t, const double* t_dev, int count, double* out, double* partial, hipStream_t s);
+
+static inline int tree_shape_max(int op, int n, int k) {
+  if (op != BM_OP_TRMEAN && op != BM_OP_PHOCAS && op != BM_OP_MEAMED) return 0;
+  if (n == 51 && k == 24) return op == BM_OP_TRMEAN ? tree_max_candidates<27, 24, BM_OP_TRMEAN>() : tree_max_candidates<27, 24, BM_OP_PHOCAS>();
+  return ((n == 11 && k == 2) || (n == 25 && (k == 5 || k == 11)) || (n == 51 && k == 12)) ? kSearchTreeMaxNodes : 0;
+}
+
+}
diff --git a/byzantinemomentum_amd/csrc/search_tree.hip b/byzantinemomentum_amd/csrc/search_tree.hip
--- /dev/null
+++ b/byzantinemomentum_amd/csrc/search_tree.hip
@@ -0,0 +1,35 @@
+#include "search_tree.h"
+
+extern "C" int bm_colwise_tree_eval_supported(int op, int n, int k) {
+  return bm::tree_shape_max(op, n, k) > 0 ? 1 : 0;
+}
+
+extern "C" int bm_colwise_tree_eval_max(int op, int n, int k) { return bm::tree_shape_max(op, n, k); }
+
+extern "C" int64_t bm_colwise_tree_eval_workspace_bytes(void) {
+  return (int64_t)bm::kSearchTreeMaxNodes * bm::kTreeCandStride * (int64_t)sizeof(double);
+}
+
+extern "C" int bm_colwise_tree_eval(int op, const float* const* honests, int h, int copies, int64_t d, int f,
+                                    const float* avg, const float* dir, const float* ts, const double* ts_dev, int count,
+                                    double* out, void* ws, void* stream) {
+  using namespace bm;
+  const int n = h + copies;
+  if (honests == nullptr || out == nullptr || ws == nullptr || h < 1 || copies < 1 || d < 0 || f != copies ||
+      count < 1 || count > tree_shape_max(op, n, copies) || (ts == nullptr) == (ts_dev == nullptr) ||
+      (d > 0 && (avg == nullptr || dir == nullptr)))
+    return BM_EINVAL;
+  for (int i = 0; i < h && d > 0; ++i)
+    if (honests[i] == nullptr) return BM_EINVAL;
+  TreeFactors t{};
+  if (ts != nullptr)
+    for (int q = 0; q < kSearchTreeMaxNodes; ++q) t.t[q] = ts[q < count ? q : count - 1];
+  double* const partial = static_cast<double*>(ws);
+  hipStream_t s = static_cast<hipStream_t>(stream);
+  switch (op) {
+    case BM_OP_TRMEAN: return launch_tree_eval_shape<BM_OP_TRMEAN>(n, copies, honests, d, avg, dir, t, ts_dev, count, out, partial, s);
+    case BM_OP_PHOCAS: return tree_eval_phocas(n, copies, honests, d, avg, dir, t, ts_dev, count, out, partial, s);
+    case BM_OP_MEAMED: return tree_eval_meamed(n, copies, honests, d, avg, dir, t, ts_dev, count, out, partial, s);
+    default: return BM_EINVAL;
+  }
+}
diff --git a/byzantinemomentum_amd/csrc/search_tree_meamed.hip b/byzantinemomentum_amd/csrc/search_tree_meamed.hip
--- /dev/null
+++ b/byzantinemomentum_amd/csrc/search_tree_meamed.hip
@@ -0,0 +1,8 @@
+#include "search_tree.h"
+
+namespace bm {
+int tree_eval_meamed(int n, int k, const float* const* rows, int64_t d, const float* avg, const float* dir,
+                     const TreeFactors& t, const double* t_dev, int count, double* out, double* partial, hipStream_t s) {
+  return launch_tree_eval_shape<BM_OP_MEAMED>(n, k, rows, d, avg, dir, t, t_dev, count, out, partial, s);
+}
+}
diff --git a/byzantinemomentum_amd/csrc/search_tree_phocas.hip b/byzantinemomentum_amd/csrc/search_tree_phocas.hip
--- /dev/null
+++ b/byzantinemomentum_amd/csrc/search_tree_phocas.hip
@@ -0,0 +1,8 @@
+#include "search_tree.h"
+
+namespace bm {
+int tree_eval_phocas(int n, int k, const float* const* rows, int64_t d, const float* avg, const float* dir,
+                     const TreeFactors& t, const double* t_dev, int count, double* out, double* partial, hipStream_t s) {
+  return launch_tree_eval_shape<BM_OP_PHOCAS>(n, k, rows, d, avg, dir, t, t_dev, count, out, partial, s);
+}
+}
diff --git a/byzantinemomentum_amd/linesearch.py b/byzantinemomentum_amd/linesearch.py
--- a/byzantinemomentum_amd/linesearch.py
+++ b/byzantinemomentum_amd/linesearch.py
@@ -21,6 +21,30 @@
     y = float(scape(x.value))
     trace.append((x.value, y))
     _lib.check(lib.bm_search_report(ctypes.byref(cursor), y), "bm_search_report")
+  return cursor.best_x, trace
+
+
+def tree_depth():
+  return int(_lib.load().bm_search_tree_depth())
+
+
+def line_maximize_tree(scape_many, evals=16, depth=3, start=0., delta=1., ratio=0.8):
+  lib = _lib.load()
+  if not isinstance(evals, int) or evals < 1 or not isinstance(depth, int) or not 1 <= depth <= 4:
+    _lib.check(_lib.EINVAL, "line_maximize_tree (evals must be a positive integer, depth 1 .. 4)")
+  cursor = _lib.Search()
+  _lib.check(lib.bm_search_begin(ctypes.byref(cursor), start, delta, ratio), "bm_search_begin")
+  trace = []
+  while cursor.evaluations < evals:
+    level = min(depth, evals - cursor.evaluations)
+    nodes = (1 << level) - 1
+    xs = (ctypes.c_double * nodes)()
+    _lib.check(lib.bm_search_tree_emit(ctypes.byref(cursor), level, ctypes.cast(xs, ctypes.c_void_p)), "bm_search_tree_emit")
+    ys = (ctypes.c_double * nodes)(*[float(y) for y in scape_many(list(xs))])
+    seen = (ctypes.c_double * (2 * level))()
+    _lib.check(lib.bm_search_tree_resolve(ctypes.byref(cursor), level, ctypes.cast(ys, ctypes.c_void_p),
+                                          ctypes.cast(seen, ctypes.c_void_p)), "bm_search_tree_resolve")
+    trace.extend((seen[2 * i], seen[2 * i + 1]) for i in range(level))
   return cursor.best_x, trace
 
 
diff --git a/byzantinemomentum_amd/sharded.py b/byzantinemomentum_amd/sharded.py
--- a/byzantinemomentum_amd/sharded.py
+++ b/byzantinemomentum_amd/sharded.py
@@ -73,7 +73,7 @@
 
   capabilities = frozenset((
     "step_worker", "momentum_stats_colwise", "momentum_stats_sqdist", "stack_stats_colwise", "stack_stats_sqdist",
-    "device_search", "attack_ranking_device", "bulyan_pass2_eval", "order_pair", "colwise_eval", "sqdist2", "anticge",
+    "device_search", "attack_ranking_device", "bulyan_pass2_eval", "order_pair", "colwise_eval", "colwise_tree_eval", "sqdist2", "anticge",
     "accept_count", "attack_vector"))
 
   def __init__(self):
@@ -193,6 +193,21 @@
 
   def colwise_eval(self, *args, **kwargs):
     return self.stats.colwise_eval(*args, **kwargs)
+
+  def colwise_tree_eval_supported(self, rule, n, copies, f):
+    return self.stats.colwise_tree_eval_supported(rule, n, copies, f)
+
+  def colwise_tree_eval_max(self, rule, n, copies, f):
+    return self.stats.colwise_tree_eval_max(rule, n, copies, f)
+
+  def colwise_tree_eval(self, *args, **kwargs):
+    return self.stats.colwise_tree_eval(*args, **kwargs)
+
+  def search_tree_depth(self):
+    return int(_lib.load().bm_search_tree_depth())
+
+  def device_tree_search(self, device, evals, negative=False, depth=3, shift=0.):
+    return self.stats.DeviceTreeSearch(device, evals, negative, depth, shift)
 
   def sqdist2(self, a, b):
     return self.stats.sqdist2(a, b)
diff --git a/byzantinemomentum_amd/stats.py b/byzantinemomentum_amd/stats.py
--- a/byzantinemomentum_amd/stats.py
+++ b/byzantinemomentum_amd/stats.py
@@ -107,6 +107,40 @@
   return out
 
 
+def colwise_tree_eval_supported(rule, n, copies, f):
+  return (rule in _EVAL_OPS and f == copies
+          and bool(_lib.load().bm_colwise_tree_eval_supported(_EVAL_OPS[rule], int(n), int(copies))))
+
+
+def colwise_tree_eval_max(rule, n, copies, f):
+  if rule not in _EVAL_OPS or f != copies:
+    return 0
+  return int(_lib.load().bm_colwise_tree_eval_max(_EVAL_OPS[rule], int(n), int(copies)))
+
+
+def colwise_tree_eval(rule, honests, copies, f, h_avg, direction, ts, count=None):
+  honests = list(honests)
+  h, d, device = gars._validate(honests)
+  gars._validate([h_avg, direction] + honests[:1])
+  lib = _lib.load()
+  on_device = isinstance(ts, torch.Tensor)
+  count = int(count if count is not None else (ts.numel() if on_device else len(ts)))
+  if not 1 <= count <= colwise_tree_eval_max(rule, h + copies, copies, f):
+    _lib.check(_lib.EINVAL, "bm_colwise_tree_eval (too many candidates)")
+  if on_device and not (ts.is_cuda and ts.device == device and ts.dtype == torch.float64 and ts.is_contiguous()
+                        and ts.numel() >= count):
+    raise gars.GarInputError("colwise_tree_eval: a tensor ts must be a contiguous float64 tensor on the vectors' device")
+  out = torch.empty(count, dtype=torch.float64, device=device)
+  ws = gars._Scratch.get(device, "ws_tree_eval", nbytes=int(lib.bm_colwise_tree_eval_workspace_bytes()))
+  host = None if on_device else (ctypes.c_float * count)(*[float(t) for t in ts])
+  with torch.cuda.device(device):
+    _lib.check(lib.bm_colwise_tree_eval(_EVAL_OPS[rule], _lib.pointer_table(honests), h, copies, d, f, _ptr(h_avg),
+                                        _ptr(direction), ctypes.cast(host, ctypes.c_void_p) if host is not None else None,
+                                        _ptr(ts) if on_device else None, count, _ptr(out), _ptr(ws),
+                                        gars._stream(device)), "bm_colwise_tree_eval")
+  return out
+
+
 def sqdist2(a, b):
   _, d, device = gars._validate([a, b])
   lib = _lib.load()
@@ -189,6 +223,43 @@
       raise RuntimeError("DeviceSearch.finish: the search has candidates left")
     self._call(y, True)
     return self.out
+
+
+class DeviceTreeSearch:
+
+  def __init__(self, device, evals, negative=False, depth=3, shift=0., start=0., delta=1., ratio=0.8):
+    if not isinstance(evals, int) or evals < 1 or not isinstance(depth, int) or not 1 <= depth <= 4:
+      _lib.check(_lib.EINVAL, "DeviceTreeSearch (evals must be a positive integer, depth 1 .. 4)")
+    self.device, self.evals, self.negative, self.depth = device, evals, bool(negative), depth
+    self.shift, self.shape = float(shift), (start, delta, ratio)
+    self.state = torch.zeros(8, dtype=torch.float64, device=device)
+    self.t = torch.zeros((1 << 4) - 1, dtype=torch.float64, device=device)
+    self.result = torch.zeros(1 + 2 * evals, dtype=torch.float64, device=device)
+    self.done = 0
+    self.started = False
+    self._nodes = 0
+    self._keep = None
+
+  def next(self, ys=None):
+    if (ys is None) == self.started:
+      raise RuntimeError("DeviceTreeSearch.next: the objectives of the last tree, None the first time")
+    level = min(self.depth, self.evals - self.done)
+    if ys is not None and not (isinstance(ys, torch.Tensor) and ys.is_cuda and ys.device == self.device
+                               and ys.dtype == torch.float64 and ys.is_contiguous()
+                               and ys.numel() >= self._nodes):
+      raise gars.GarInputError("DeviceTreeSearch: the objectives must be a float64 tensor on the search's device")
+    lib = _lib.load()
+    self._keep = ys
+    with torch.cuda.device(self.device):
+      _lib.check(lib.bm_search_device_tree_next(_ptr(self.state), _opt(ys), 1 if self.negative else 0, self.shift,
+                                                self.depth, self.evals, *self.shape, _ptr(self.t), _ptr(self.result),
+                                                gars._stream(self.device)), "bm_search_device_tree_next")
+    self.started = True
+    if level <= 0:
+      return None
+    self.done += level
+    self._nodes = (1 << level) - 1
+    return self.t, self._nodes
 
 
 def study_stats(s_avg, h_avg, defense, byz, f_real, past_newest=None, curv=None, past_oldest=None, curv_mode=0, mu=0.0,
diff --git a/byzantinemomentum_amd/step.py b/byzantinemomentum_amd/step.py
--- a/byzantinemomentum_amd/step.py
+++ b/byzantinemomentum_amd/step.py
@@ -214,6 +214,27 @@
       self.agg.all_reduce_sum(sq)
       return sq
 
+    many = getattr(evaluate, "many", None)
+    depth = min(self.ops.search_tree_depth(), evaluate.many_depth) if many is not None else 1
+    if depth > 1 and on_device:
+      cursor = self.ops.device_tree_search(h_avg.device, self.attack_evals, self.attack_negative, depth, shift)
+      ys = None
+      while True:
+        tree = cursor.next(ys)
+        if tree is None:
+          break
+        ys = many(*tree)
+        self.agg.all_reduce_sum(ys)
+      found = self.last_search = cursor.result
+      return found
+    if depth > 1:
+      def objectives(xs):
+        ts = [(-x if self.attack_negative else x) for x in xs]
+        ys = many([t + shift if shift else t for t in ts], len(ts))
+        self.agg.all_reduce_sum(ys)
+        return self._fetch(ys).tolist()
+      factor, self.last_search = linesearch.line_maximize_tree(objectives, evals=self.attack_evals, depth=depth)
+      return factor
     if on_device:
       cursor = self.ops.device_search(h_avg.device, self.attack_evals, self.attack_negative)
       y = None
@@ -264,7 +285,13 @@
     ops, k = self.ops, self.f_real
     if not ops.colwise_eval_supported(self.gar, self.h + k):
       return self._generic_objective(honests, h_avg, direction)
-    return lambda t: ops.colwise_eval(self.gar, honests, k, self.f_decl, h_avg, direction, t)
+    def evaluate(t):
+      return ops.colwise_eval(self.gar, honests, k, self.f_decl, h_avg, direction, t)
+    if ("colwise_tree_eval" in self.plan.capabilities
+        and ops.colwise_tree_eval_supported(self.gar, self.h + k, k, self.f_decl)):
+      evaluate.many = lambda ts, count: ops.colwise_tree_eval(self.gar, honests, k, self.f_decl, h_avg, direction, ts, count)
+      evaluate.many_depth = (ops.colwise_tree_eval_max(self.gar, self.h + k, k, self.f_decl) + 1).bit_length() - 1
+    return evaluate
 
   def _median_objective(self, honests, h_avg, direction, on_device=False):
     ops, agg, h, k = self.ops, self.agg, self.h, self.f_real
diff --git a/include/bm_gar.h b/include/bm_gar.h
--- a/include/bm_gar.h
+++ b/include/bm_gar.h
@@ -21,6 +21,7 @@
 
 int bm_abi_version(void);
 int bm_tuning_set(const char* name, int value);
+int bm_search_tree_depth(void);
 
 const char* bm_error_string(int code);
 
@@ -184,6 +185,13 @@
 int bm_colwise_eval_tdev(int op, const float* const* honests, int h, int copies, int64_t d, int f, const float* avg,
                          const float* dir, const double* t_dev, double* out, void* ws, void* stream);
 
+int bm_colwise_tree_eval_supported(int op, int n, int copies);
+int bm_colwise_tree_eval_max(int op, int n, int copies);
+int64_t bm_colwise_tree_eval_workspace_bytes(void);
+int bm_colwise_tree_eval(int op, const float* const* honests, int h, int copies, int64_t d, int f, const float* avg,
+                         const float* dir, const float* ts, const double* ts_dev, int count, double* out, void* ws,
+                         void* stream);
+
 typedef struct bm_search {
   double best_x, best_y;
   double probe;
@@ -196,6 +204,8 @@
 int bm_search_begin(bm_search* c, double start, double delta, double ratio);
 int bm_search_propose(bm_search* c, double* x_out);
 int bm_search_report(bm_search* c, double y);
+int bm_search_tree_emit(const bm_search* c, int depth, double* xs_out);
+int bm_search_tree_resolve(bm_search* c, int depth, const double* ys, double* trace_out);
 int bm_attack_objective(const double* ext, int h, int k, int f, int rule, int m, double t, double* y_out,
                         int32_t* sel_out, int32_t* count_out);
 int bm_attack_line_search(const double* ext, int h, int k, int f, int rule, int m, int evals, int negative,
@@ -213,6 +223,8 @@
 int bm_order_pair(const float* const* rows, int h, int64_t d, int il, int ih, float* lo, float* hi, void* stream);
 int bm_search_device_next(void* state, const double* y, int negative, int last, double start, double delta, double ratio,
                           double* t_out, double* out, void* stream);
+int bm_search_device_tree_next(void* state, const double* ys, int negative, double shift, int depth, int evals,
+                               double start, double delta, double ratio, double* t_out, double* out, void* stream);
 int bm_attack_ranking(const double* ext, int h, int k, int f, int mode, int m, double t, int32_t* order_out);
 
 #ifdef __cplusplus
```

Result: no change. 5154 (-0.2%).
